# GDMCF/GDMCF

Measured on AMD Instinct MI355X. Metric: training users/sec, higher is better.
Workload: dtype f32; 1 GPU; yelp-shape synthetic rows, batch=400/GPU, dims=[1000], T=5, noise_scale=0.01, linear-var, mean_type=x0, reweight, AdamW lr=1e-5 (BASELINE configs[1]); n_items=34395, global_batch=400, parallelism=dp1, batch_rows=device CSR rows (CsrBatch)

## Files before the change

### gdmcf_amd/build.py

```python
import concurrent.futures
import hashlib
import os
import re
import subprocess
import sys

CSRC = os.path.join(os.path.dirname(os.path.abspath(__file__)), "csrc")
SOURCES = ["capi.hip", "dp_exchange.hip", "gemm_f32.hip", "gemm_bf16.hip", "gemm_split.hip", "gemm_small.hip", "gemm_dr.hip", "gemm_dr_tn.hip", "gemm_dr_fat.hip", "gemm_dr_kn.hip", "prep_input.hip", "noise.hip", "loss_tail.hip", "adamw.hip", "rows.hip", "reduce.hip", "linear.hip", "topk_spmm.hip", "spmm_bundle.hip", "score_topk.hip", "score_rank.hip", "bpr.hip", "cat.hip", "gather_fwd.hip", "ntxent.hip", "latent_step.hip", "cand_scores.hip", "rank.hip"]
HEADERS = ["common.h", "draws.h", "rank_order.h", "score_product.h", "gemm_dr.h", "gemm_epilogue.h", os.path.join("..", "..", "include", "gdmcf_hip.h")]
LIB = os.path.join(CSRC, "libgdmcf_hip.so")
ASM_LINT = ("gemm_dr_tn.hip", "gemm_split.hip")
STORE_LINT = ("gemm_f32.hip", "gemm_bf16.hip", "gemm_dr_fat.hip", "gemm_dr_kn.hip", "score_topk.hip", "score_rank.hip", "latent_step.hip")
NO_SPILL = ("gemm_f32.hip", "gemm_bf16.hip", "gemm_split.hip", "gemm_dr_tn.hip", "score_topk.hip", "score_rank.hip", "cat.hip", "gather_fwd.hip", "ntxent.hip", "latent_step.hip", "cand_scores.hip")
FLAGS = ["--offload-arch=gfx950", "-O3", "-std=c++17", "-fPIC", "-Wall", "-Wno-unused-function"]


def _hipcc():
    for c in (os.environ.get("HIPCC"), "/opt/rocm/bin/hipcc", "hipcc"):
        if c and (os.path.isabs(c) and os.path.exists(c) or not os.path.isabs(c)):
            return c
    raise RuntimeError("hipcc not found")


def _digest():
    h = hashlib.sha256()
    for f in SOURCES + HEADERS:
        with open(os.path.join(CSRC, f), "rb") as fh:
            h.update(fh.read())
    h.update(" ".join(FLAGS).encode())
    return h.hexdigest()


_REG = re.compile(r"\bv(\d+)\b|\bv\[(\d+):(\d+)\]")


def _regs(text):
    out = set()
    for m in _REG.finditer(text):
        if m.group(1) is not None:
            out.add(int(m.group(1)))
        else:
            out.update(range(int(m.group(2)), int(m.group(3)) + 1))
    return out


_SREG = re.compile(r"\bs(\d+)\b|\bs\[(\d+):(\d+)\]")


def _sregs(text):
    out = set()
    for m in _SREG.finditer(text):
        if m.group(1) is not None:
            out.add(int(m.group(1)))
        else:
            out.update(range(int(m.group(2)), int(m.group(3)) + 1))
    return out


def lint_ring_registers(asm_text, kernel_prefix="dr_tn_kernel"):
    bad, seen = [], 0
    for m in re.finditer(r"^(\S*%s\S*):[^\n]*\n(.*?)\n\s*s_endpgm" % kernel_prefix, asm_text, flags=re.S | re.M):
        name, body = m.group(1), m.group(2)
        seen += 1
        lines = [ln.split(";")[0].strip() for ln in body.splitlines()]
        lines = [ln for ln in lines if ln and not ln.endswith(":") and not ln.startswith(".")]
        ring = set()
        for ln in lines:
            if ln.startswith("buffer_load_dwordx4"):
                ring |= _regs(ln.split(",")[0])
        if not ring:
            bad.append(f"{name}: no asm ring loads found (lint out of date?)")
            continue
        first = next(i for i, ln in enumerate(lines) if ln.startswith("buffer_load_dwordx4"))
        drains = [i for i, ln in enumerate(lines) if ln.startswith("s_waitcnt") and "vmcnt(0)" in ln]
        last = drains[-1] if drains and drains[-1] > first else len(lines)
        for ln in lines[first:last]:
            mnem, _, ops = ln.partition(" ")
            parts = [o.strip() for o in ops.split(",")]
            if mnem.startswith("buffer_load_dwordx4"):
                if _regs(",".join(parts[1:])) & ring:
                    bad.append(f"{name}: ring register used as an address: {ln}")
            elif mnem.startswith("v_mfma"):
                if (_regs(parts[0]) | _regs(parts[3] if len(parts) > 3 else "")) & ring:
                    bad.append(f"{name}: MFMA accumulator inside the operand ring: {ln}")
            elif mnem.startswith(("v_mov", "v_pk_mov", "v_accvgpr", "scratch_", "v_swap")):
                if _regs(ops) & ring:
                    bad.append(f"{name}: copy or spill of a ring register: {ln}")
    if not seen:
        bad.append(f"no function named *{kernel_prefix}* in the assembly (lint out of date?)")
    return bad


_COPY = ("v_mov", "v_pk_mov", "v_accvgpr", "scratch_", "v_swap")
_VMEM = ("buffer_", "global_", "flat_", "scratch_")


def lint_vmcnt(asm_text, only=None):
    bad, nk = [], 0
    for m in re.finditer(r"^(_Z\S+):[^\n]*\n(.*?)\n\s*s_endpgm", asm_text, flags=re.S | re.M):
        name, body = m.group(1), m.group(2)
        if only and only not in name:
            continue
        ins, in_asm = [], False
        for ln in body.splitlines():
            t = ln.strip()
            if t.startswith(";;#ASMSTART"):
                in_asm = True
                continue
            if t.startswith(";;#ASMEND"):
                in_asm = False
                continue
            c = t.split(";")[0].strip()
            if not c or (c.startswith(".") and not c.endswith(":")):
                continue
            ins.append((c, in_asm))
        if not any(a and "load_dword" in c.split()[0] for c, a in ins):
            continue
        nk += 1
        leaders, labels = {0}, {}
        for k, (c, a) in enumerate(ins):
            if c.endswith(":"):
                labels[c[:-1]] = k
                leaders.add(k)
            elif c.startswith(("s_cbranch", "s_branch")):
                leaders.add(k + 1)
        starts = sorted(x for x in leaders if x < len(ins))
        blocks = [(st, starts[i + 1] if i + 1 < len(starts) else len(ins)) for i, st in enumerate(starts)]
        blk_of = {st: i for i, (st, en) in enumerate(blocks)}
        succ = []
        for bi, (st, en) in enumerate(blocks):
            mn, _, ops = ins[en - 1][0].partition(" ")
            nxt = []
            if mn.startswith(("s_cbranch", "s_branch")) and labels.get(ops.strip()) is not None:
                nxt.append(blk_of[labels[ops.strip()]])
            if not mn.startswith("s_branch") and bi + 1 < len(blocks):
                nxt.append(bi + 1)
            succ.append(nxt)
        found = {}

        def transfer(bi, st_in, report):
            st = dict(st_in)
            fresh = {}
            for k in range(*blocks[bi]):
                ln, a = ins[k]
                if ln.endswith(":"):
                    continue
                mnem, _, ops = ln.partition(" ")
                parts = [o.strip() for o in ops.split(",")]
                if a and mnem.startswith(_VMEM):
                    hot = _sregs(ops) & fresh.keys()
                    if hot and report:
                        found.setdefault(f"s{min(hot)} written by a VALU instruction < 5 wait states before this asm load reads it: {ln}", k)
                step = int(ops) + 1 if mnem == "s_nop" and ops.strip().isdigit() else 1
                fresh = {r: w - step for r, w in fresh.items() if w - step > 0}
                if mnem.startswith("v_") and parts and re.fullmatch(r"s\d+|s\[\d+:\d+\]", parts[0]):
                    for r in _sregs(parts[0]):
                        fresh[r] = 5
                if mnem == "s_waitcnt":
                    mm = re.search(r"vmcnt\((\d+)\)", ops)
                    if mm:
                        st = {r: rk for r, rk in st.items() if rk < int(mm.group(1))}
                    continue
                asm_load = a and "load_dword" in mnem
                touched = _regs(",".join(parts[1:]) if asm_load else ops) & st.keys()
                if touched and report:
                    what = "used as an address" if asm_load else ("copied / spilled" if mnem.startswith(_COPY) else "used")
                    found.setdefault(f"register v{min(touched)} {what} before a counted wait covers its load: {ln}", k)
                if mnem.startswith(_VMEM):
                    st = {r: min(rk + 1, 64) for r, rk in st.items()}
                    if asm_load:
                        for r in _regs(parts[0]):
                            st[r] = 0
            return st

        state = [None] * len(blocks)
        state[0] = {}
        work = [0]
        while work:
            bi = work.pop()
            out = transfer(bi, state[bi], False)
            for sj in succ[bi]:
                if state[sj] is None:
                    state[sj] = dict(out)
                    work.append(sj)
                else:
                    changed = False
                    for r, rk in out.items():
                        if state[sj].get(r, 65) > rk:
                            state[sj][r] = rk
                            changed = True
                    if changed:
                        work.append(sj)
        for bi in range(len(blocks)):
            if state[bi] is not None:
                transfer(bi, state[bi], True)
        bad += [f"{name}: {msg}" for msg, k in sorted(found.items(), key=lambda kv: kv[1])]
    if not nk:
        bad.append("no kernel with inline-asm loads in the assembly (lint out of date?)")
    return bad


def lint_store_data(asm_text):
    bad = []
    for m in re.finditer(r"^(_Z\S+):[^\n]*\n(.*?)\n\s*s_endpgm", asm_text, flags=re.S | re.M):
        name, body = m.group(1), m.group(2)
        lines = [ln.split(";")[0].strip() for ln in body.splitlines()]
        lines = [ln for ln in lines if ln and not ln.startswith(".") and not ln.endswith(":")]
        for k, ln in enumerate(lines):
            mnem, _, ops = ln.partition(" ")
            if not re.match(r"(buffer|global|flat|scratch)_store_dwordx[34]$", mnem):
                continue
            parts = [o.strip() for o in ops.split(",")]
            data = _regs(parts[1] if mnem.startswith(("global", "flat", "scratch")) else parts[0])
            left = 2
            for nxt in lines[k + 1:k + 8]:
                nm, _, nops = nxt.partition(" ")
                if nm == "s_nop":
                    left -= int(nops.strip() or 0) + 1
                else:
                    nparts = [o.strip() for o in nops.split(",")]
                    if nm.startswith("v_") and nparts and _regs(nparts[0]) & data and left > 0:
                        bad.append(f"{name}: data register of `{ln}` rewritten {2 - left} wait state(s) later by `{nxt}`")
                        break
                    left -= 1
                if left <= 0:
                    break
    return bad


def lint_fat_dma(asm_text, kernel="dr_fat_kernel"):
    bad, n_dma = [], 0
    for m in re.finditer(r"^(_Z\S*%s\S*):[^\n]*\n(.*?)\n\s*s_endpgm" % kernel, asm_text, flags=re.S | re.M):
        name, body = m.group(1), m.group(2)
        lines = [ln.split(";")[0].strip() for ln in body.splitlines()]
        lines = [ln for ln in lines if ln and (not ln.startswith(".") or ln.endswith(":"))]
        if not any(ln.startswith("buffer_load_dwordx4") and ln.endswith(" lds") for ln in lines):
            continue
        n_dma += 1
        pending = None
        for ln in lines:
            if ln.startswith("buffer_load_dwordx4") and ln.endswith(" lds"):
                pending = ln
            elif ln.startswith("s_waitcnt") and re.search(r"vmcnt\(0\)", ln):
                pending = None
            elif ln.startswith("ds_read_b128") and pending:
                bad.append(f"{name}: `{ln}` follows `{pending}` with no s_waitcnt vmcnt(0) in between")
                break
        loops, label, blk = 0, None, []
        for ln in lines + ["end:"]:
            if not ln.endswith(":"):
                blk.append(ln)
                continue
            if label and any(i.startswith("v_mfma") for i in blk) and any(
                    i.startswith(("s_cbranch", "s_branch")) and i.split()[-1] == label for i in blk):
                loops += 1
                moved = [i for i in blk if i.startswith(("scratch_", "v_accvgpr", "v_mov"))]
                if moved:
                    bad.append(f"{name}: {len(moved)} spill / move instruction(s) in the k loop, e.g. `{moved[0]}`")
            label, blk = ln[:-1], []
        if not loops:
            bad.append(f"{name}: no k loop found (lint out of date?)")
    if not n_dma:
        bad.append(f"no *{kernel}* with `buffer_load_dwordx4 ... lds` in the assembly (lint out of date?)")
    return bad


def build(force=False, verbose=True):
    stamp = os.path.join(CSRC, ".build_stamp")
    dig = _digest()
    if not force and os.path.exists(LIB) and os.path.exists(stamp) and open(stamp).read() == dig:
        return LIB
    hipcc = _hipcc()
    objs = []

    def compile_one(src):
        obj = os.path.join(CSRC, src.replace(".hip", ".o"))
        cmd = [hipcc] + FLAGS + ["-c", os.path.join(CSRC, src), "-o", obj]
        guarded = src in NO_SPILL
        if guarded:
            cmd.append("-Rpass-analysis=kernel-resource-usage")
        r = subprocess.run(cmd, capture_output=True, text=True)
        if r.returncode != 0:
            raise RuntimeError(f"hipcc failed for {src}:\n{r.stderr}")
        err = r.stderr
        if guarded:
            name, bad = None, []
            for line in err.splitlines():
                if "Function Name:" in line:
                    name = line.split("Function Name:")[1].split()[0]
                elif "VGPRs Spill:" in line and int(line.split("VGPRs Spill:")[1].split()[0]) > 0:
                    bad.append(name)
            if bad:
                raise RuntimeError(f"{src}: register spills in {len(bad)} kernel(s) with uncounted asm loads, e.g. {bad[0]}")
            err = err if ("warning:" in err or "error:" in err) else ""
        if verbose and err.strip():
            print(err, file=sys.stderr)
        if src in ASM_LINT or src in STORE_LINT:
            asm = os.path.join(CSRC, src.replace(".hip", ".lint.s"))
            r2 = subprocess.run([hipcc] + FLAGS + ["-S", "--cuda-device-only", os.path.join(CSRC, src), "-o", asm],
                                capture_output=True, text=True)
            if r2.returncode != 0:
                raise RuntimeError(f"hipcc -S failed for {src}:\n{r2.stderr}")
            text = open(asm).read()
            os.remove(asm)
            bad = lint_store_data(text)
            if src in ASM_LINT:
                bad += lint_vmcnt(text)
            if src == "gemm_dr_tn.hip":
                bad += lint_ring_registers(text)
            if src == "gemm_dr_fat.hip":
                bad += lint_fat_dma(text)
            if bad:
                raise RuntimeError(f"{src}: ISA lint failed (lint_store_data / lint_vmcnt / lint_ring_registers / lint_fat_dma):\n  " + "\n  ".join(bad[:12]))
        return obj

    with concurrent.futures.ThreadPoolExecutor(max_workers=min(8, len(SOURCES))) as ex:
        objs = list(ex.map(compile_one, SOURCES))
    cmd = [hipcc, "--offload-arch=gfx950", "-shared", "-fPIC", "-o", LIB] + objs
    r = subprocess.run(cmd, capture_output=True, text=True)
    if r.returncode != 0:
        raise RuntimeError(f"link failed:\n{r.stderr}")
    with open(stamp, "w") as fh:
        fh.write(dig)
    if verbose:
        print(f"built {LIB}")
    return LIB


if __name__ == "__main__":
    build(force="--force" in sys.argv)
```

### gdmcf_amd/csrc/gemm_dr.h

```cpp
#pragma once

#include "common.h"

namespace {
struct DrArgs {
    GdGemm g;
    int tiles_m, tiles_n, m_fastest;
    int ksp;
    int ctr;
    const GdAdamHyper* adam_dev;
    int stagger;
};
}

struct DrRoutes {
    bool dw;
    bool adamw;
    bool kn;
    bool fat;
    bool fat_slab;
};
DrRoutes& dr_routes();
int dr_cu_count();
int dr_stagger();

int gd_dr_tn_launch(GdGemm& g, hipStream_t s);
int gd_dr_kn_launch(GdGemm& g, hipStream_t s);
int gd_dr_fat_launch(int epi, GdGemm& g, hipStream_t s);
int gd_dr_fat_slab_launch(GdGemm& g, hipStream_t s);
```

### gdmcf_amd/csrc/gemm_dr.hip

```cpp
#include <stdlib.h>

#include "gemm_dr.h"

int dr_cu_count() {
    static int n_cu = 0;
    if (n_cu == 0) {
        int dev = 0;
        hipDeviceProp_t prop;
        n_cu = (hipGetDevice(&dev) == hipSuccess && hipGetDeviceProperties(&prop, dev) == hipSuccess) ? prop.multiProcessorCount : 256;
    }
    return n_cu;
}

#ifndef GD_FAT_SLAB_DEFAULT
#define GD_FAT_SLAB_DEFAULT 1
#endif

static bool dr_env_on(const char* name, bool dflt = true) {
    const char* v = getenv(name);
    return v == nullptr ? dflt : atoi(v) != 0;
}
DrRoutes& dr_routes() {
    static DrRoutes r = {dr_env_on("GDMCF_DR_DW"), dr_env_on("GDMCF_DR_ADAMW"), dr_env_on("GDMCF_DR_KN"), dr_env_on("GDMCF_DR_FAT"),
                         dr_env_on("GDMCF_DR_FAT_SLAB", GD_FAT_SLAB_DEFAULT != 0)};
    return r;
}

int dr_stagger() {
    static const int stagger = getenv("GDMCF_DR_STAGGER") ? atoi(getenv("GDMCF_DR_STAGGER")) : 3;
    return stagger;
}

int gd_gemm_dr_launch(int layA, int layB, int epi, GdGemm& g, hipStream_t s) {
    if (g.bf16) return GD_DR_NOT_TAKEN;
    if (g.accumulate || g.C16 || (g.splits > 1 && epi != GD_EPI_SLAB)) return GD_DR_NOT_TAKEN;
    if (layA == GD_LAY_MC && layB == GD_LAY_MC) {
        if (epi == GD_EPI_ADAMW) return gd_gemm_dr_adamw_multi(&g, 1, s);
        if (epi == GD_EPI_STORE) return gd_dr_tn_launch(g, s);
    } else if (layA == GD_LAY_KC && layB == GD_LAY_MC) {
        if (epi == GD_EPI_SLAB) return gd_dr_kn_launch(g, s);
    } else if (layA == GD_LAY_KC && layB == GD_LAY_KC) {
        if (epi == GD_EPI_LOSS || epi == GD_EPI_POST) return gd_dr_fat_launch(epi, g, s);
        if (epi == GD_EPI_SLAB) return gd_dr_fat_slab_launch(g, s);
    }
    return GD_DR_NOT_TAKEN;
}
```

### gdmcf_amd/csrc/gemm_dr_fat.hip

```cpp
#include <stdlib.h>

#include "gemm_dr.h"

#ifndef GD_FAT_DMA_DEFAULT
#define GD_FAT_DMA_DEFAULT 1
#endif

namespace {

template <int NB, int EPI, int DMA>
__global__ __launch_bounds__(256, 1) void dr_fat_kernel(const DrArgs d) {
    static_assert(EPI == GD_EPI_LOSS || EPI == GD_EPI_POST || EPI == GD_EPI_SLAB, "output layer with a fused epilogue, or split-K slabs");
    static_assert(NB >= 4 && NB <= 12, "5 x NB accumulator blocks must fit 256 registers");
    static_assert(DMA == 0 || DMA == 1, "B through staging registers, or straight into LDS");
    constexpr bool SLAB = EPI == GD_EPI_SLAB;
    typedef __attribute__((address_space(3))) void* lds_vp;
    constexpr int WAIT_VM0 = 0x0F70, WAIT_LGKM0 = 0xC07F;
    constexpr int TMB = 5;
    const GdGemm& g = d.g;
    const int lane = threadIdx.x & 63;
    const int wave = __builtin_amdgcn_readfirstlane(threadIdx.x >> 6);
    const int r = lane & 15, q = lane >> 4;
    extern __shared__ __attribute__((aligned(16))) float dr_lds[];
    float* const lds = dr_lds + wave * (2 * NB * 256);
    const int nblk = gridDim.x, per = nblk >> 3;
    const int wl = ((nblk & 7) == 0 ? ((int)(blockIdx.x & 7) * per + (int)(blockIdx.x >> 3)) : (int)blockIdx.x) * 4 + wave;
    const int n_waves = nblk * 4;
    const int ntiles = d.tiles_m * d.tiles_n;
    const __amdgpu_buffer_rsrc_t srdA = __builtin_amdgcn_make_buffer_rsrc(const_cast<float*>(g.A), 0, (int)(((int64_t)(g.M - 1) * g.lda + g.K) * 4), 0x00020000);
    const __amdgpu_buffer_rsrc_t srdB = __builtin_amdgcn_make_buffer_rsrc(const_cast<float*>(g.B), 0, (int)(((int64_t)(g.N - 1) * g.ldb + g.K) * 4), 0x00020000);
    const int NCH = d.ksp;
    const int c_mask = g.K >> 4;
    const int ntasks = SLAB ? ntiles * g.splits : ntiles;
    const int w_off = (lane >> 2) * 16 + (((lane & 3) ^ ((((lane >> 2) >> 2) & 1) << 1)) << 2);
    const int g_slot = DMA ? ((lane & 3) ^ ((((lane >> 2) >> 2) & 1) << 1)) : (lane & 3);
    const int r_off = r * 16 + ((q ^ (((r >> 2) & 1) << 1)) << 2);
    for (int task = wl; task < ntasks; task += n_waves) {
        const int split = SLAB ? task / ntiles : 0;
        const int tile = SLAB ? task - split * ntiles : task;
        const int c_lo = SLAB ? split * (g.kchunk >> 4) : 0;
        const int c_hi = SLAB ? min(c_lo + (g.kchunk >> 4), NCH) : NCH;
        const int c_in = SLAB ? min(c_hi, c_mask) : c_mask;
        const int tm = tile % d.tiles_m, tn = tile / d.tiles_m;
        const int m0 = tm * (16 * TMB), n0 = tn * (16 * NB);
        uint32_t offA[TMB], offB[NB];
#pragma unroll
        for (int i = 0; i < TMB; ++i) offA[i] = (uint32_t)((m0 + 16 * i + r) * g.lda + 4 * q) * 4u;
#pragma unroll
        for (int p = 0; p < NB; ++p) offB[p] = (uint32_t)(((int64_t)(n0 + 16 * p + (lane >> 2)) * g.ldb + 4 * g_slot) * 4);
        f32x4 acc[TMB][NB];
#pragma unroll
        for (int i = 0; i < TMB; ++i)
#pragma unroll
            for (int b = 0; b < NB; ++b) acc[i][b] = f32x4{0.f, 0.f, 0.f, 0.f};
        f32x4 xa[2][TMB], G[DMA ? 1 : NB], FB[NB];
        const int hp = DMA ? ((c_in - c_lo) & 1) : 0;
        const int k_lo = SLAB ? c_lo * 64 : 0;
        if (hp) {
#pragma unroll
            for (int i = 0; i < TMB; ++i) xa[1][i] = __builtin_bit_cast(f32x4, __builtin_amdgcn_raw_buffer_load_b128(srdA, offA[i], k_lo, 0));
        } else {
#pragma unroll
            for (int i = 0; i < TMB; ++i) xa[0][i] = __builtin_bit_cast(f32x4, __builtin_amdgcn_raw_buffer_load_b128(srdA, offA[i], k_lo, 0));
        }
        if constexpr (DMA) {
            __builtin_amdgcn_sched_barrier(0);
            __builtin_amdgcn_s_waitcnt(WAIT_LGKM0);
            __builtin_amdgcn_sched_barrier(0);
#pragma unroll
            for (int p = 0; p < NB; ++p) __builtin_amdgcn_raw_ptr_buffer_load_lds(srdB, (lds_vp)(lds + hp * (NB * 256) + p * 256), 16, (int)offB[p], k_lo, 0, 0);
        } else {
#pragma unroll
            for (int p = 0; p < NB; ++p) G[p] = __builtin_bit_cast(f32x4, __builtin_amdgcn_raw_buffer_load_b128(srdB, offB[p], k_lo, 0));
#pragma unroll
            for (int p = 0; p < NB; ++p) *reinterpret_cast<f32x4*>(lds + p * 256 + w_off) = G[p];
        }

#define GD_FAT_CHUNK(PAR, c, MSK)                                                                                         \
        {                                                                                                             \
             \
            const uint32_t kn = ((c) + 1 < c_hi) ? (uint32_t)((c) + 1) * 64u : 0x80000000u;                           \
            if constexpr (DMA) {                                                                                      \
                __builtin_amdgcn_sched_barrier(0);                                                                    \
                __builtin_amdgcn_s_waitcnt(WAIT_VM0);                                                                 \
                __builtin_amdgcn_sched_barrier(0);                                                                    \
            }                                                                                                         \
            _Pragma("unroll") for (int b = 0; b < NB; ++b)                                                            \
                FB[b] = *reinterpret_cast<const f32x4*>(lds + (PAR) * (NB * 256) + b * 256 + r_off);                  \
            if (MSK) {  \
                 \
                _Pragma("unroll") for (int e = 0; e < 4; ++e) {                                                       \
                    const bool keep = (c) * 16 + 4 * q + e < g.K;                                                     \
                    _Pragma("unroll") for (int i = 0; i < TMB; ++i) xa[PAR][i][e] = keep ? xa[PAR][i][e] : 0.f;       \
                    _Pragma("unroll") for (int b = 0; b < NB; ++b) FB[b][e] = keep ? FB[b][e] : 0.f;                  \
                }                                                                                                     \
            }                                                                                                         \
            __builtin_amdgcn_sched_barrier(0);                                                                        \
            _Pragma("unroll") for (int sx = 0; sx < 4; ++sx) {                                                        \
                _Pragma("unroll") for (int n = 0; n < TMB * NB; ++n) {                                                \
                    const int i = n / NB, b = n % NB;                                                                 \
                    if (sx == 0 && i == 0) asm volatile("" : "+v"(FB[b]));  \
                    if (sx == 0 && b == 0) asm volatile("" : "+v"(xa[PAR][i]));                                       \
                    acc[i][b] = __builtin_amdgcn_mfma_f32_16x16x4f32(xa[PAR][i][sx], FB[b][sx], acc[i][b], 0, 0, 0);  \
                     \
                    if (sx < 2 && n % 5 == 2) {      \
                        const int l = (sx == 0) ? n / 5 : NB + n / 5;                                                 \
                        if (l < TMB + NB) {                                                                           \
                            __builtin_amdgcn_sched_barrier(0);                                                        \
                            if (l < TMB)                                                                              \
                                xa[(PAR) ^ 1][l] = __builtin_bit_cast(f32x4, __builtin_amdgcn_raw_buffer_load_b128(   \
                                    srdA, offA[l], kn, 0));                                                           \
                            else if constexpr (DMA)                                                                   \
                                __builtin_amdgcn_raw_ptr_buffer_load_lds(                                             \
                                    srdB, (lds_vp)(lds + ((PAR) ^ 1) * (NB * 256) + (l - TMB) * 256), 16,             \
                                    (int)offB[l - TMB], (int)kn, 0, 0);                                               \
                            else                                                                                      \
                                G[l - TMB] = __builtin_bit_cast(f32x4, __builtin_amdgcn_raw_buffer_load_b128(         \
                                    srdB, offB[l - TMB], kn, 0));                                                     \
                            __builtin_amdgcn_sched_barrier(0);                                                        \
                        }                                                                                             \
                    }                                                                                                 \
                    if (!DMA && sx == 3 && n % 4 == 1 && n / 4 < NB) {  \
                        __builtin_amdgcn_sched_barrier(0);                                                            \
                        *reinterpret_cast<f32x4*>(lds + ((PAR) ^ 1) * (NB * 256) + (n / 4) * 256 + w_off) = G[n / 4]; \
                        __builtin_amdgcn_sched_barrier(0);                                                            \
                    }                                                                                                 \
                }                                                                                                     \
                __builtin_amdgcn_sched_barrier(0);                                                                    \
            }                                                                                                         \
        }
        const int c_pf = d.stagger > 0 ? ((NCH > d.stagger + 2 ? NCH - d.stagger : 0) & ~1) : -2;
        const int c_pairs = DMA ? c_in : c_hi;
        const int c_pfl = (DMA && c_pf >= 0) ? min(c_pf | hp, c_pairs - 2) : c_pf;
        int c = c_lo;
        if constexpr (DMA) {
            if (hp) {
                GD_FAT_CHUNK(1, c_lo, false);
                c = c_lo + 1;
            }
        }
        for (; c + 1 < c_pairs; c += 2) {
            if constexpr (EPI == GD_EPI_POST) {
                if (c == c_pfl) {
                    constexpr int NJL = (16 * NB * 4 + 127) / 128 + 1;
                    constexpr int NPI = (80 * NJL + 63) / 64;
                    float* const scratch = dr_lds + 4 * (2 * NB * 256) + wave * 64;
                    const __amdgpu_buffer_rsrc_t srdX = __builtin_amdgcn_make_buffer_rsrc(
                        const_cast<float*>(g.aux), 0, (int)(((int64_t)(g.M - 1) * g.ldaux + g.N) * 4), 0x00020000);
#pragma unroll
                    for (int pi = 0; pi < NPI; ++pi) {
                        const int t = min(pi * 64 + lane, 80 * NJL - 1);
                        const int row = min(m0 + t % 80, g.M - 1), j = t / 80;
                        const int col = min(j < NJL - 1 ? n0 + 32 * j : n0 + 16 * NB - 1, g.N - 1);
                        __builtin_amdgcn_raw_ptr_buffer_load_lds(srdX, (lds_vp)scratch, 4, (int)(((int64_t)row * g.ldaux + col) * 4), 0, 0, 0);
                    }
                }
            }
            if constexpr (DMA) {
                GD_FAT_CHUNK(0, c, false);
                GD_FAT_CHUNK(1, c + 1, false);
            } else {
                GD_FAT_CHUNK(0, c, c >= c_mask);
                GD_FAT_CHUNK(1, c + 1, c + 1 >= c_mask);
            }
        }
        if constexpr (DMA) {
            if (c < c_hi) GD_FAT_CHUNK(0, c, true);
        } else {
            if ((c_hi - c_lo) & 1) GD_FAT_CHUNK(0, c_hi - 1, c_hi - 1 >= c_mask);
        }
#undef GD_FAT_CHUNK
        if constexpr (DMA) {
            __builtin_amdgcn_sched_barrier(0);
            __builtin_amdgcn_s_waitcnt(WAIT_VM0);
            __builtin_amdgcn_sched_barrier(0);
        }

        if constexpr (SLAB) {
            constexpr int LDS_S = 16 * NB + 4, NJ_S = (4 * NB + 15) / 16;
            float* const slab = g.C + (int64_t)split * g.slab_stride;
#pragma unroll
            for (int i = 0; i < TMB; ++i) {
#pragma unroll
                for (int b = 0; b < NB; ++b)
#pragma unroll
                    for (int t = 0; t < 4; ++t) lds[(4 * q + t) * LDS_S + 16 * b + r] = acc[i][b][t];
                __builtin_amdgcn_sched_barrier(0);
#pragma unroll
                for (int p4 = 0; p4 < 4; ++p4) {
                    const int m = m0 + 16 * i + 4 * p4 + q;
#pragma unroll
                    for (int j = 0; j < NJ_S; ++j) {
                        const int c4 = r + 16 * j;
                        const int n = n0 + 4 * c4;
                        const f32x4 v = *reinterpret_cast<const f32x4*>(lds + (4 * p4 + q) * LDS_S + 4 * min(c4, 4 * NB - 1));
                        if (c4 < 4 * NB && m < g.M) {
                            if (n + 3 < g.N) {
                                *reinterpret_cast<f32x4*>(slab + (int64_t)m * g.ldc + n) = v;
                            } else {
                                for (int e = 0; e < 4 && n + e < g.N; ++e) slab[(int64_t)m * g.ldc + n + e] = v[e];
                            }
                        }
                    }
                }
                __builtin_amdgcn_sched_barrier(0);
            }
            continue;
        }

        constexpr int LDS_ = 16 * NB + 4;
        constexpr int NJ = (4 * NB + 15) / 16;
        typedef f32x4 f32x4_e __attribute__((aligned(4)));
        f32x4 bias4[NJ];
        int col4[NJ];
#pragma unroll
        for (int j = 0; j < NJ; ++j) {
            col4[j] = n0 + 4 * (r + 16 * j);
            bias4[j] = f32x4{0.f, 0.f, 0.f, 0.f};
            if (g.bias && r + 16 * j < 4 * NB) {
#pragma unroll
                for (int e = 0; e < 4; ++e) bias4[j][e] = g.bias[min(col4[j] + e, g.N - 1)];
            }
        }
        const bool has_z = (EPI == GD_EPI_POST) && (g.aux2 != nullptr);
        const bool has_r = (EPI == GD_EPI_POST) && (g.r2 != nullptr);
        struct Pre {
            f32x4 a[NJ], z[NJ];
            uint32_t w[NJ];
            float c1, c2, p1, p2, sg;
        } pre[2];
        auto fetch = [&](int i, int p4, Pre& P) {
            const int mc = min(m0 + 16 * i + 4 * p4 + q, g.M - 1);
            P.c1 = 1.f; P.c2 = 0.f; P.p1 = 0.f; P.p2 = 0.f; P.sg = 0.f;
            if (EPI == GD_EPI_LOSS) {
                if (g.r0) P.c1 = g.r0[mc];
            } else {
                P.c1 = g.r0[mc];
                P.c2 = g.r1[mc];
                if (has_r) { P.p1 = g.r2[mc]; P.p2 = g.r3[mc]; }
                if (has_z) P.sg = g.r4[mc];
            }
#pragma unroll
            for (int j = 0; j < NJ; ++j) {
                const int n = col4[j];
                const bool whole = (r + 16 * j < 4 * NB) && n + 3 < g.N;
                P.w[j] = 0u;
                P.a[j] = f32x4{0.f, 0.f, 0.f, 0.f};
                P.z[j] = f32x4{0.f, 0.f, 0.f, 0.f};
                if (EPI == GD_EPI_LOSS && g.aux_bits) {
                    P.w[j] = g.aux_bits[(int64_t)mc * g.ldbits + min((int64_t)(n >> 5), g.ldbits - 1)];
                } else if (whole) {
                    P.a[j] = *reinterpret_cast<const f32x4_e*>(g.aux + (int64_t)mc * g.ldaux + n);
                    if (has_z) P.z[j] = *reinterpret_cast<const f32x4_e*>(g.aux2 + (int64_t)mc * g.ldaux2 + n);
                }
            }
        };
        fetch(0, 0, pre[0]);
#pragma unroll
        for (int i = 0; i < TMB; ++i) {
#pragma unroll
            for (int b = 0; b < NB; ++b)
#pragma unroll
                for (int t = 0; t < 4; ++t) lds[(4 * q + t) * LDS_ + 16 * b + r] = acc[i][b][t];
            __builtin_amdgcn_sched_barrier(0);
#pragma unroll
            for (int p4 = 0; p4 < 4; ++p4) {
                const int step = 4 * i + p4;
                const Pre& P = pre[step & 1];
                if (step + 1 < 4 * TMB) fetch((step + 1) >> 2, (step + 1) & 3, pre[(step + 1) & 1]);
                const int m = m0 + 16 * i + 4 * p4 + q;
                const int mc = min(m, g.M - 1);
                const bool mok = m < g.M;
                float ss = 0.f;
                const float c1 = P.c1, c2 = P.c2, p1 = P.p1, p2 = P.p2, sg = P.sg;
#pragma unroll
                for (int j = 0; j < NJ; ++j) {
                    const int c4 = r + 16 * j;
                    const bool inb = c4 < 4 * NB;
                    const int n = col4[j];
                    const bool whole = inb && n + 3 < g.N;
                    const bool full = whole && mok;
                    const f32x4 v = *reinterpret_cast<const f32x4*>(lds + (4 * p4 + q) * LDS_ + 4 * min(c4, 4 * NB - 1));
                    f32x4 o, o2 = f32x4{0.f, 0.f, 0.f, 0.f};
                    if (EPI == GD_EPI_LOSS) {
                        f32x4 tg;
                        if (g.aux_bits) {
                            const uint32_t w = P.w[j] >> (n & 31);
#pragma unroll
                            for (int e = 0; e < 4; ++e) tg[e] = (float)((w >> e) & 1u);
                        } else if (whole) {
                            tg = P.a[j];
                        } else {
#pragma unroll
                            for (int e = 0; e < 4; ++e) tg[e] = g.aux[(int64_t)mc * g.ldaux + min(n + e, g.N - 1)];
                        }
#pragma unroll
                        for (int e = 0; e < 4; ++e) {
                            o2[e] = v[e] + bias4[j][e];
                            o[e] = c1 * o2[e] - tg[e];
                            if (inb && mok && n + e < g.N) ss += o[e] * o[e];
                        }
                    } else {
                        f32x4 xt = P.a[j], zz = P.z[j];
                        if (!whole) {
#pragma unroll
                            for (int e = 0; e < 4; ++e) {
                                xt[e] = g.aux[(int64_t)mc * g.ldaux + min(n + e, g.N - 1)];
                                if (has_z) zz[e] = g.aux2[(int64_t)mc * g.ldaux2 + min(n + e, g.N - 1)];
                            }
                        }
#pragma unroll
                        for (int e = 0; e < 4; ++e) {
                            const float vv = v[e] + bias4[j][e];
                            o2[e] = has_r ? (p1 * xt[e] - p2 * vv) : vv;
                            o[e] = c1 * o2[e] + c2 * xt[e];
                            if (has_z) o[e] += sg * zz[e];
                        }
                    }
                    if (full) {
                        *reinterpret_cast<f32x4_e*>(g.C + (int64_t)m * g.ldc + n) = o;
                        if (g.out2) *reinterpret_cast<f32x4_e*>(g.out2 + (int64_t)m * g.ldout2 + n) = o2;
                    } else if (inb && mok) {
                        for (int e = 0; e < 4 && n + e < g.N; ++e) {
                            g.C[(int64_t)m * g.ldc + n + e] = o[e];
                            if (g.out2) g.out2[(int64_t)m * g.ldout2 + n + e] = o2[e];
                        }
                    }
                }
                if (EPI == GD_EPI_LOSS) {
                    ss += __shfl_xor(ss, 1);
                    ss += __shfl_xor(ss, 2);
                    ss += __shfl_xor(ss, 4);
                    ss += __shfl_xor(ss, 8);
                    if (r == 0 && mok) g.rowpart[(int64_t)m * g.ld_rowpart + tn] = ss;
                }
                __builtin_amdgcn_sched_barrier(0);
            }
        }
    }
}

template <int NB>
int dr_fat_go(const DrArgs& d, int epi, int dma, int n_cu, hipStream_t s) {
    const size_t lds = (size_t)4 * 2 * NB * 256 * sizeof(float) + 4 * 64 * sizeof(float);
    void (*kern)(const DrArgs) =
        dma ? (epi == GD_EPI_SLAB ? dr_fat_kernel<NB, GD_EPI_SLAB, 1> : epi == GD_EPI_LOSS ? dr_fat_kernel<NB, GD_EPI_LOSS, 1> : dr_fat_kernel<NB, GD_EPI_POST, 1>)
            : (epi == GD_EPI_SLAB ? dr_fat_kernel<NB, GD_EPI_SLAB, 0> : epi == GD_EPI_LOSS ? dr_fat_kernel<NB, GD_EPI_LOSS, 0> : dr_fat_kernel<NB, GD_EPI_POST, 0>);
    static bool attr_set[6] = {false, false, false, false, false, false};
    const int ai = epi == GD_EPI_SLAB ? 4 + dma : 2 * dma + (epi == GD_EPI_LOSS);
    if (!attr_set[ai] && lds > 48 * 1024) {
        hipError_t e = hipFuncSetAttribute(reinterpret_cast<const void*>(kern), hipFuncAttributeMaxDynamicSharedMemorySize, (int)lds);
        if (e != hipSuccess) {
            gdmcf_set_error("hipFuncSetAttribute(dr_fat_kernel, LDS=%zu): %s", lds, hipGetErrorString(e));
            return GDMCF_E_HIP;
        }
        attr_set[ai] = true;
    }
    hipLaunchKernelGGL(kern, dim3(n_cu), dim3(256), lds, s, d);
    return GDMCF_OK;
}

int dr_fat_dma(const GdGemm& g) {
    static const int dma_env = getenv("GDMCF_FAT_DMA") ? atoi(getenv("GDMCF_FAT_DMA")) : GD_FAT_DMA_DEFAULT;
    return (dma_env > 0 && (reinterpret_cast<uintptr_t>(g.B) & 15) == 0 && (g.ldb & 3) == 0) ? 1 : 0;
}

}

int gd_dr_fat_launch(int epi, GdGemm& g, hipStream_t s) {
    if (!dr_routes().fat) return GD_DR_NOT_TAKEN;
    const int64_t lim = (int64_t)1 << 32;
    const int n_cu = dr_cu_count();
    const int tiles_m = gd_cdiv(g.M, 80);
    bool ok = (int64_t)g.M * g.lda * 4 < ((int64_t)1 << 31) && (int64_t)g.N * g.ldb * 4 < lim && g.lda >= g.K && g.ldb >= g.K &&
              g.K >= 256 && (long)tiles_m * 80 * 100 <= (long)g.M * 112 &&
              (n_cu & 7) == 0 && !(epi == GD_EPI_LOSS && g.rowpart == nullptr) &&
              !(epi == GD_EPI_LOSS && g.aux_bits && g.ldbits < (g.N + 31) / 32);
    int nb = 0;
    long best = 1L << 60;
    const long slots = 4L * n_cu;
    for (int c = 12; c >= 8 && ok; --c) {
        const long t = (long)tiles_m * gd_cdiv(g.N, 16 * c);
        const long cost = ((t + slots - 1) / slots) * c;
        if (t >= slots / 2 && cost < best) { best = cost; nb = c; }
    }
    if (ok && epi == GD_EPI_POST) {
        const long t128 = (long)gd_cdiv(g.M, 80) * gd_cdiv(g.N, 128);
        const long rounds = (t128 + 2 * n_cu - 1) / (2 * n_cu);
        if (t128 * 100 >= rounds * 2 * n_cu * 90) ok = false;
    }
    if (!ok || !nb || (epi == GD_EPI_LOSS && g.ld_rowpart < gd_cdiv(g.N, 16 * nb))) return GD_DR_NOT_TAKEN;
    DrArgs d = {};
    d.tiles_m = tiles_m;
    d.tiles_n = gd_cdiv(g.N, 16 * nb);
    d.m_fastest = 1;
    d.ksp = gd_cdiv(g.K, 16);
    {
        static const int pf = getenv("GDMCF_FAT_PF") ? atoi(getenv("GDMCF_FAT_PF")) : 10;
        d.stagger = pf;
    }
    const int dma = dr_fat_dma(g);
    g.tiles_m = d.tiles_m;
    g.tiles_n = d.tiles_n;
    d.g = g;
    d.ctr = 0;
    int rc = GDMCF_OK;
    {
        GdProfScope prof(g.prof_tag, 2.0 * g.M * g.N * g.K, s);
        switch (nb) {
            case 8: rc = dr_fat_go<8>(d, epi, dma, n_cu, s); break;
            case 9: rc = dr_fat_go<9>(d, epi, dma, n_cu, s); break;
            case 10: rc = dr_fat_go<10>(d, epi, dma, n_cu, s); break;
            case 11: rc = dr_fat_go<11>(d, epi, dma, n_cu, s); break;
            default: rc = dr_fat_go<12>(d, epi, dma, n_cu, s); break;
        }
    }
    if (rc != GDMCF_OK) return rc;
    t_gd_last_gemm = 4;
    return gd_launch_status("gemm_dr");
}

int gd_dr_fat_slab_plan(int M, int N, int K, int* nb_out, int* cps_out) {
    if (!dr_routes().fat_slab || M <= 0 || N < 128 || K < 4096) return 0;
    const int n_cu = dr_cu_count();
    const int tiles_m = gd_cdiv(M, 80);
    if ((n_cu & 7) != 0 || (long)tiles_m * 80 * 100 > (long)M * 112) return 0;
    const long slots = 4L * n_cu;
    const int chunks = gd_cdiv(K, 16);
    int nb = 0, cps = 0;
    long best = 1L << 60;
    for (int c = 8; c <= 12; ++c) {
        const long tiles = (long)tiles_m * gd_cdiv(N, 16 * c);
        if (tiles > slots) continue;
        long sp = slots / tiles;
        if (sp > chunks / 8) sp = chunks / 8;
        if (sp > 64) sp = 64;
        if (sp < 2) continue;
        const int per = gd_cdiv(chunks, (int)sp);
        if ((long)c * per < best) { best = (long)c * per; nb = c; cps = per; }
    }
    if (!nb) return 0;
    if (nb_out) *nb_out = nb;
    if (cps_out) *cps_out = cps;
    return gd_cdiv(chunks, cps);
}

int gd_dr_fat_slab_launch(GdGemm& g, hipStream_t s) {
    int nb = 0, cps = 0;
    const int splits = gd_dr_fat_slab_plan(g.M, g.N, g.K, &nb, &cps);
    if (!splits) return GD_DR_NOT_TAKEN;
    const size_t need = (size_t)splits * g.M * g.ldc * sizeof(float);
    const bool ok = gd_aligned16(g.C) && (g.ldc & 3) == 0 && g.ldc >= g.N &&
                    g.ws_cap >= need && g.slab_stride >= (int64_t)g.M * g.ldc && (g.slab_stride & 3) == 0 &&
                    (int64_t)g.M * g.lda * 4 < ((int64_t)1 << 31) && (int64_t)g.N * g.ldb * 4 < ((int64_t)1 << 32) && g.lda >= g.K && g.ldb >= g.K;
    if (!ok) return GD_DR_NOT_TAKEN;
    const int n_cu = dr_cu_count();
    DrArgs d = {};
    d.tiles_m = gd_cdiv(g.M, 80);
    d.tiles_n = gd_cdiv(g.N, 16 * nb);
    d.m_fastest = 1;
    d.ksp = gd_cdiv(g.K, 16);
    g.splits = splits;
    g.kchunk = cps * 16;
    g.tiles_m = d.tiles_m;
    g.tiles_n = d.tiles_n;
    d.g = g;
    d.ctr = 0;
    const int dma = dr_fat_dma(g);
    int rc = GDMCF_OK;
    {
        GdProfScope prof(g.prof_tag, 2.0 * g.M * g.N * g.K, s);
        switch (nb) {
            case 8: rc = dr_fat_go<8>(d, GD_EPI_SLAB, dma, n_cu, s); break;
            case 9: rc = dr_fat_go<9>(d, GD_EPI_SLAB, dma, n_cu, s); break;
            case 10: rc = dr_fat_go<10>(d, GD_EPI_SLAB, dma, n_cu, s); break;
            case 11: rc = dr_fat_go<11>(d, GD_EPI_SLAB, dma, n_cu, s); break;
            default: rc = dr_fat_go<12>(d, GD_EPI_SLAB, dma, n_cu, s); break;
        }
    }
    if (rc != GDMCF_OK) return rc;
    t_gd_last_gemm = 6;
    return gd_launch_status("gemm_dr_fat_slab");
}
```

Before: 321,100 users/s.

## Specialize fat GEMM epilogues by feature flags and split into separate compilation units

Moves the fat output-layer GEMM kernel into a shared header and adds a template flag parameter that selects specialized LOSS/POST epilogue variants, including an interior-tile fast path and software-prefetched per-row epilogue operands. The instantiations are split across new source files so they compile in parallel. The aim is to cut branching and the exposed latency of global loads in the fused epilogue for the output layer. In exchange it brings more template instantiations, longer build times and a larger code size, and the epilogue logic is duplicated across variants.

```diff
diff --git a/gdmcf_amd/build.py b/gdmcf_amd/build.py
--- a/gdmcf_amd/build.py
+++ b/gdmcf_amd/build.py
@@ -6,11 +6,11 @@
 import sys
 
 CSRC = os.path.join(os.path.dirname(os.path.abspath(__file__)), "csrc")
-SOURCES = ["capi.hip", "dp_exchange.hip", "gemm_f32.hip", "gemm_bf16.hip", "gemm_split.hip", "gemm_small.hip", "gemm_dr.hip", "gemm_dr_tn.hip", "gemm_dr_fat.hip", "gemm_dr_kn.hip", "prep_input.hip", "noise.hip", "loss_tail.hip", "adamw.hip", "rows.hip", "reduce.hip", "linear.hip", "topk_spmm.hip", "spmm_bundle.hip", "score_topk.hip", "score_rank.hip", "bpr.hip", "cat.hip", "gather_fwd.hip", "ntxent.hip", "latent_step.hip", "cand_scores.hip", "rank.hip"]
-HEADERS = ["common.h", "draws.h", "rank_order.h", "score_product.h", "gemm_dr.h", "gemm_epilogue.h", os.path.join("..", "..", "include", "gdmcf_hip.h")]
+SOURCES = ["capi.hip", "dp_exchange.hip", "gemm_f32.hip", "gemm_bf16.hip", "gemm_split.hip", "gemm_small.hip", "gemm_dr.hip", "gemm_dr_tn.hip", "gemm_dr_fat.hip", "gemm_dr_fat_loss.hip", "gemm_dr_fat_post.hip", "gemm_dr_fat_post2.hip", "gemm_dr_kn.hip", "prep_input.hip", "noise.hip", "loss_tail.hip", "adamw.hip", "rows.hip", "reduce.hip", "linear.hip", "topk_spmm.hip", "spmm_bundle.hip", "score_topk.hip", "score_rank.hip", "bpr.hip", "cat.hip", "gather_fwd.hip", "ntxent.hip", "latent_step.hip", "cand_scores.hip", "rank.hip"]
+HEADERS = ["common.h", "draws.h", "rank_order.h", "score_product.h", "gemm_dr.h", "gemm_dr_fat_kernel.h", "gemm_epilogue.h", os.path.join("..", "..", "include", "gdmcf_hip.h")]
 LIB = os.path.join(CSRC, "libgdmcf_hip.so")
 ASM_LINT = ("gemm_dr_tn.hip", "gemm_split.hip")
-STORE_LINT = ("gemm_f32.hip", "gemm_bf16.hip", "gemm_dr_fat.hip", "gemm_dr_kn.hip", "score_topk.hip", "score_rank.hip", "latent_step.hip")
+STORE_LINT = ("gemm_f32.hip", "gemm_bf16.hip", "gemm_dr_fat.hip", "gemm_dr_fat_loss.hip", "gemm_dr_fat_post.hip", "gemm_dr_fat_post2.hip", "gemm_dr_kn.hip", "score_topk.hip", "score_rank.hip", "latent_step.hip")
 NO_SPILL = ("gemm_f32.hip", "gemm_bf16.hip", "gemm_split.hip", "gemm_dr_tn.hip", "score_topk.hip", "score_rank.hip", "cat.hip", "gather_fwd.hip", "ntxent.hip", "latent_step.hip", "cand_scores.hip")
 FLAGS = ["--offload-arch=gfx950", "-O3", "-std=c++17", "-fPIC", "-Wall", "-Wno-unused-function"]
 
@@ -308,7 +308,7 @@
                 bad += lint_vmcnt(text)
             if src == "gemm_dr_tn.hip":
                 bad += lint_ring_registers(text)
-            if src == "gemm_dr_fat.hip":
+            if src.startswith("gemm_dr_fat"):
                 bad += lint_fat_dma(text)
             if bad:
                 raise RuntimeError(f"{src}: ISA lint failed (lint_store_data / lint_vmcnt / lint_ring_registers / lint_fat_dma):\n  " + "\n  ".join(bad[:12]))
diff --git a/gdmcf_amd/csrc/gemm_dr.h b/gdmcf_amd/csrc/gemm_dr.h
--- a/gdmcf_amd/csrc/gemm_dr.h
+++ b/gdmcf_amd/csrc/gemm_dr.h
@@ -10,6 +10,7 @@
     int ctr;
     const GdAdamHyper* adam_dev;
     int stagger;
+    int interior;
 };
 }
 
@@ -19,6 +20,7 @@
     bool kn;
     bool fat;
     bool fat_slab;
+    bool fat_epi;
 };
 DrRoutes& dr_routes();
 int dr_cu_count();
diff --git a/gdmcf_amd/csrc/gemm_dr.hip b/gdmcf_amd/csrc/gemm_dr.hip
--- a/gdmcf_amd/csrc/gemm_dr.hip
+++ b/gdmcf_amd/csrc/gemm_dr.hip
@@ -16,13 +16,17 @@
 #define GD_FAT_SLAB_DEFAULT 1
 #endif
 
+#ifndef GD_FAT_EPI_DEFAULT
+#define GD_FAT_EPI_DEFAULT 1
+#endif
+
 static bool dr_env_on(const char* name, bool dflt = true) {
     const char* v = getenv(name);
     return v == nullptr ? dflt : atoi(v) != 0;
 }
 DrRoutes& dr_routes() {
     static DrRoutes r = {dr_env_on("GDMCF_DR_DW"), dr_env_on("GDMCF_DR_ADAMW"), dr_env_on("GDMCF_DR_KN"), dr_env_on("GDMCF_DR_FAT"),
-                         dr_env_on("GDMCF_DR_FAT_SLAB", GD_FAT_SLAB_DEFAULT != 0)};
+                         dr_env_on("GDMCF_DR_FAT_SLAB", GD_FAT_SLAB_DEFAULT != 0), dr_env_on("GDMCF_FAT_EPI", GD_FAT_EPI_DEFAULT != 0)};
     return r;
 }
 
diff --git a/gdmcf_amd/csrc/gemm_dr_fat.hip b/gdmcf_amd/csrc/gemm_dr_fat.hip
--- a/gdmcf_amd/csrc/gemm_dr_fat.hip
+++ b/gdmcf_amd/csrc/gemm_dr_fat.hip
@@ -1,6 +1,6 @@
 #include <stdlib.h>
 
-#include "gemm_dr.h"
+#include "gemm_dr_fat_kernel.h"
 
 #ifndef GD_FAT_DMA_DEFAULT
 #define GD_FAT_DMA_DEFAULT 1
@@ -8,356 +8,11 @@
 
 namespace {
 
-template <int NB, int EPI, int DMA>
-__global__ __launch_bounds__(256, 1) void dr_fat_kernel(const DrArgs d) {
-    static_assert(EPI == GD_EPI_LOSS || EPI == GD_EPI_POST || EPI == GD_EPI_SLAB, "output layer with a fused epilogue, or split-K slabs");
-    static_assert(NB >= 4 && NB <= 12, "5 x NB accumulator blocks must fit 256 registers");
-    static_assert(DMA == 0 || DMA == 1, "B through staging registers, or straight into LDS");
-    constexpr bool SLAB = EPI == GD_EPI_SLAB;
-    typedef __attribute__((address_space(3))) void* lds_vp;
-    constexpr int WAIT_VM0 = 0x0F70, WAIT_LGKM0 = 0xC07F;
-    constexpr int TMB = 5;
-    const GdGemm& g = d.g;
-    const int lane = threadIdx.x & 63;
-    const int wave = __builtin_amdgcn_readfirstlane(threadIdx.x >> 6);
-    const int r = lane & 15, q = lane >> 4;
-    extern __shared__ __attribute__((aligned(16))) float dr_lds[];
-    float* const lds = dr_lds + wave * (2 * NB * 256);
-    const int nblk = gridDim.x, per = nblk >> 3;
-    const int wl = ((nblk & 7) == 0 ? ((int)(blockIdx.x & 7) * per + (int)(blockIdx.x >> 3)) : (int)blockIdx.x) * 4 + wave;
-    const int n_waves = nblk * 4;
-    const int ntiles = d.tiles_m * d.tiles_n;
-    const __amdgpu_buffer_rsrc_t srdA = __builtin_amdgcn_make_buffer_rsrc(const_cast<float*>(g.A), 0, (int)(((int64_t)(g.M - 1) * g.lda + g.K) * 4), 0x00020000);
-    const __amdgpu_buffer_rsrc_t srdB = __builtin_amdgcn_make_buffer_rsrc(const_cast<float*>(g.B), 0, (int)(((int64_t)(g.N - 1) * g.ldb + g.K) * 4), 0x00020000);
-    const int NCH = d.ksp;
-    const int c_mask = g.K >> 4;
-    const int ntasks = SLAB ? ntiles * g.splits : ntiles;
-    const int w_off = (lane >> 2) * 16 + (((lane & 3) ^ ((((lane >> 2) >> 2) & 1) << 1)) << 2);
-    const int g_slot = DMA ? ((lane & 3) ^ ((((lane >> 2) >> 2) & 1) << 1)) : (lane & 3);
-    const int r_off = r * 16 + ((q ^ (((r >> 2) & 1) << 1)) << 2);
-    for (int task = wl; task < ntasks; task += n_waves) {
-        const int split = SLAB ? task / ntiles : 0;
-        const int tile = SLAB ? task - split * ntiles : task;
-        const int c_lo = SLAB ? split * (g.kchunk >> 4) : 0;
-        const int c_hi = SLAB ? min(c_lo + (g.kchunk >> 4), NCH) : NCH;
-        const int c_in = SLAB ? min(c_hi, c_mask) : c_mask;
-        const int tm = tile % d.tiles_m, tn = tile / d.tiles_m;
-        const int m0 = tm * (16 * TMB), n0 = tn * (16 * NB);
-        uint32_t offA[TMB], offB[NB];
-#pragma unroll
-        for (int i = 0; i < TMB; ++i) offA[i] = (uint32_t)((m0 + 16 * i + r) * g.lda + 4 * q) * 4u;
-#pragma unroll
-        for (int p = 0; p < NB; ++p) offB[p] = (uint32_t)(((int64_t)(n0 + 16 * p + (lane >> 2)) * g.ldb + 4 * g_slot) * 4);
-        f32x4 acc[TMB][NB];
-#pragma unroll
-        for (int i = 0; i < TMB; ++i)
-#pragma unroll
-            for (int b = 0; b < NB; ++b) acc[i][b] = f32x4{0.f, 0.f, 0.f, 0.f};
-        f32x4 xa[2][TMB], G[DMA ? 1 : NB], FB[NB];
-        const int hp = DMA ? ((c_in - c_lo) & 1) : 0;
-        const int k_lo = SLAB ? c_lo * 64 : 0;
-        if (hp) {
-#pragma unroll
-            for (int i = 0; i < TMB; ++i) xa[1][i] = __builtin_bit_cast(f32x4, __builtin_amdgcn_raw_buffer_load_b128(srdA, offA[i], k_lo, 0));
-        } else {
-#pragma unroll
-            for (int i = 0; i < TMB; ++i) xa[0][i] = __builtin_bit_cast(f32x4, __builtin_amdgcn_raw_buffer_load_b128(srdA, offA[i], k_lo, 0));
-        }
-        if constexpr (DMA) {
-            __builtin_amdgcn_sched_barrier(0);
-            __builtin_amdgcn_s_waitcnt(WAIT_LGKM0);
-            __builtin_amdgcn_sched_barrier(0);
-#pragma unroll
-            for (int p = 0; p < NB; ++p) __builtin_amdgcn_raw_ptr_buffer_load_lds(srdB, (lds_vp)(lds + hp * (NB * 256) + p * 256), 16, (int)offB[p], k_lo, 0, 0);
-        } else {
-#pragma unroll
-            for (int p = 0; p < NB; ++p) G[p] = __builtin_bit_cast(f32x4, __builtin_amdgcn_raw_buffer_load_b128(srdB, offB[p], k_lo, 0));
-#pragma unroll
-            for (int p = 0; p < NB; ++p) *reinterpret_cast<f32x4*>(lds + p * 256 + w_off) = G[p];
-        }
-
-#define GD_FAT_CHUNK(PAR, c, MSK)                                                                                         \
-        {                                                                                                             \
-             \
-            const uint32_t kn = ((c) + 1 < c_hi) ? (uint32_t)((c) + 1) * 64u : 0x80000000u;                           \
-            if constexpr (DMA) {                                                                                      \
-                __builtin_amdgcn_sched_barrier(0);                                                                    \
-                __builtin_amdgcn_s_waitcnt(WAIT_VM0);                                                                 \
-                __builtin_amdgcn_sched_barrier(0);                                                                    \
-            }                                                                                                         \
-            _Pragma("unroll") for (int b = 0; b < NB; ++b)                                                            \
-                FB[b] = *reinterpret_cast<const f32x4*>(lds + (PAR) * (NB * 256) + b * 256 + r_off);                  \
-            if (MSK) {  \
-                 \
-                _Pragma("unroll") for (int e = 0; e < 4; ++e) {                                                       \
-                    const bool keep = (c) * 16 + 4 * q + e < g.K;                                                     \
-                    _Pragma("unroll") for (int i = 0; i < TMB; ++i) xa[PAR][i][e] = keep ? xa[PAR][i][e] : 0.f;       \
-                    _Pragma("unroll") for (int b = 0; b < NB; ++b) FB[b][e] = keep ? FB[b][e] : 0.f;                  \
-                }                                                                                                     \
-            }                                                                                                         \
-            __builtin_amdgcn_sched_barrier(0);                                                                        \
-            _Pragma("unroll") for (int sx = 0; sx < 4; ++sx) {                                                        \
-                _Pragma("unroll") for (int n = 0; n < TMB * NB; ++n) {                                                \
-                    const int i = n / NB, b = n % NB;                                                                 \
-                    if (sx == 0 && i == 0) asm volatile("" : "+v"(FB[b]));  \
-                    if (sx == 0 && b == 0) asm volatile("" : "+v"(xa[PAR][i]));                                       \
-                    acc[i][b] = __builtin_amdgcn_mfma_f32_16x16x4f32(xa[PAR][i][sx], FB[b][sx], acc[i][b], 0, 0, 0);  \
-                     \
-                    if (sx < 2 && n % 5 == 2) {      \
-                        const int l = (sx == 0) ? n / 5 : NB + n / 5;                                                 \
-                        if (l < TMB + NB) {                                                                           \
-                            __builtin_amdgcn_sched_barrier(0);                                                        \
-                            if (l < TMB)                                                                              \
-                                xa[(PAR) ^ 1][l] = __builtin_bit_cast(f32x4, __builtin_amdgcn_raw_buffer_load_b128(   \
-                                    srdA, offA[l], kn, 0));                                                           \
-                            else if constexpr (DMA)                                                                   \
-                                __builtin_amdgcn_raw_ptr_buffer_load_lds(                                             \
-                                    srdB, (lds_vp)(lds + ((PAR) ^ 1) * (NB * 256) + (l - TMB) * 256), 16,             \
-                                    (int)offB[l - TMB], (int)kn, 0, 0);                                               \
-                            else                                                                                      \
-                                G[l - TMB] = __builtin_bit_cast(f32x4, __builtin_amdgcn_raw_buffer_load_b128(         \
-                                    srdB, offB[l - TMB], kn, 0));                                                     \
-                            __builtin_amdgcn_sched_barrier(0);                                                        \
-                        }                                                                                             \
-                    }                                                                                                 \
-                    if (!DMA && sx == 3 && n % 4 == 1 && n / 4 < NB) {  \
-                        __builtin_amdgcn_sched_barrier(0);                                                            \
-                        *reinterpret_cast<f32x4*>(lds + ((PAR) ^ 1) * (NB * 256) + (n / 4) * 256 + w_off) = G[n / 4]; \
-                        __builtin_amdgcn_sched_barrier(0);                                                            \
-                    }                                                                                                 \
-                }                                                                                                     \
-                __builtin_amdgcn_sched_barrier(0);                                                                    \
-            }                                                                                                         \
-        }
-        const int c_pf = d.stagger > 0 ? ((NCH > d.stagger + 2 ? NCH - d.stagger : 0) & ~1) : -2;
-        const int c_pairs = DMA ? c_in : c_hi;
-        const int c_pfl = (DMA && c_pf >= 0) ? min(c_pf | hp, c_pairs - 2) : c_pf;
-        int c = c_lo;
-        if constexpr (DMA) {
-            if (hp) {
-                GD_FAT_CHUNK(1, c_lo, false);
-                c = c_lo + 1;
-            }
-        }
-        for (; c + 1 < c_pairs; c += 2) {
-            if constexpr (EPI == GD_EPI_POST) {
-                if (c == c_pfl) {
-                    constexpr int NJL = (16 * NB * 4 + 127) / 128 + 1;
-                    constexpr int NPI = (80 * NJL + 63) / 64;
-                    float* const scratch = dr_lds + 4 * (2 * NB * 256) + wave * 64;
-                    const __amdgpu_buffer_rsrc_t srdX = __builtin_amdgcn_make_buffer_rsrc(
-                        const_cast<float*>(g.aux), 0, (int)(((int64_t)(g.M - 1) * g.ldaux + g.N) * 4), 0x00020000);
-#pragma unroll
-                    for (int pi = 0; pi < NPI; ++pi) {
-                        const int t = min(pi * 64 + lane, 80 * NJL - 1);
-                        const int row = min(m0 + t % 80, g.M - 1), j = t / 80;
-                        const int col = min(j < NJL - 1 ? n0 + 32 * j : n0 + 16 * NB - 1, g.N - 1);
-                        __builtin_amdgcn_raw_ptr_buffer_load_lds(srdX, (lds_vp)scratch, 4, (int)(((int64_t)row * g.ldaux + col) * 4), 0, 0, 0);
-                    }
-                }
-            }
-            if constexpr (DMA) {
-                GD_FAT_CHUNK(0, c, false);
-                GD_FAT_CHUNK(1, c + 1, false);
-            } else {
-                GD_FAT_CHUNK(0, c, c >= c_mask);
-                GD_FAT_CHUNK(1, c + 1, c + 1 >= c_mask);
-            }
-        }
-        if constexpr (DMA) {
-            if (c < c_hi) GD_FAT_CHUNK(0, c, true);
-        } else {
-            if ((c_hi - c_lo) & 1) GD_FAT_CHUNK(0, c_hi - 1, c_hi - 1 >= c_mask);
-        }
-#undef GD_FAT_CHUNK
-        if constexpr (DMA) {
-            __builtin_amdgcn_sched_barrier(0);
-            __builtin_amdgcn_s_waitcnt(WAIT_VM0);
-            __builtin_amdgcn_sched_barrier(0);
-        }
-
-        if constexpr (SLAB) {
-            constexpr int LDS_S = 16 * NB + 4, NJ_S = (4 * NB + 15) / 16;
-            float* const slab = g.C + (int64_t)split * g.slab_stride;
-#pragma unroll
-            for (int i = 0; i < TMB; ++i) {
-#pragma unroll
-                for (int b = 0; b < NB; ++b)
-#pragma unroll
-                    for (int t = 0; t < 4; ++t) lds[(4 * q + t) * LDS_S + 16 * b + r] = acc[i][b][t];
-                __builtin_amdgcn_sched_barrier(0);
-#pragma unroll
-                for (int p4 = 0; p4 < 4; ++p4) {
-                    const int m = m0 + 16 * i + 4 * p4 + q;
-#pragma unroll
-                    for (int j = 0; j < NJ_S; ++j) {
-                        const int c4 = r + 16 * j;
-                        const int n = n0 + 4 * c4;
-                        const f32x4 v = *reinterpret_cast<const f32x4*>(lds + (4 * p4 + q) * LDS_S + 4 * min(c4, 4 * NB - 1));
-                        if (c4 < 4 * NB && m < g.M) {
-                            if (n + 3 < g.N) {
-                                *reinterpret_cast<f32x4*>(slab + (int64_t)m * g.ldc + n) = v;
-                            } else {
-                                for (int e = 0; e < 4 && n + e < g.N; ++e) slab[(int64_t)m * g.ldc + n + e] = v[e];
-                            }
-                        }
-                    }
-                }
-                __builtin_amdgcn_sched_barrier(0);
-            }
-            continue;
-        }
-
-        constexpr int LDS_ = 16 * NB + 4;
-        constexpr int NJ = (4 * NB + 15) / 16;
-        typedef f32x4 f32x4_e __attribute__((aligned(4)));
-        f32x4 bias4[NJ];
-        int col4[NJ];
-#pragma unroll
-        for (int j = 0; j < NJ; ++j) {
-            col4[j] = n0 + 4 * (r + 16 * j);
-            bias4[j] = f32x4{0.f, 0.f, 0.f, 0.f};
-            if (g.bias && r + 16 * j < 4 * NB) {
-#pragma unroll
-                for (int e = 0; e < 4; ++e) bias4[j][e] = g.bias[min(col4[j] + e, g.N - 1)];
-            }
-        }
-        const bool has_z = (EPI == GD_EPI_POST) && (g.aux2 != nullptr);
-        const bool has_r = (EPI == GD_EPI_POST) && (g.r2 != nullptr);
-        struct Pre {
-            f32x4 a[NJ], z[NJ];
-            uint32_t w[NJ];
-            float c1, c2, p1, p2, sg;
-        } pre[2];
-        auto fetch = [&](int i, int p4, Pre& P) {
-            const int mc = min(m0 + 16 * i + 4 * p4 + q, g.M - 1);
-            P.c1 = 1.f; P.c2 = 0.f; P.p1 = 0.f; P.p2 = 0.f; P.sg = 0.f;
-            if (EPI == GD_EPI_LOSS) {
-                if (g.r0) P.c1 = g.r0[mc];
-            } else {
-                P.c1 = g.r0[mc];
-                P.c2 = g.r1[mc];
-                if (has_r) { P.p1 = g.r2[mc]; P.p2 = g.r3[mc]; }
-                if (has_z) P.sg = g.r4[mc];
-            }
-#pragma unroll
-            for (int j = 0; j < NJ; ++j) {
-                const int n = col4[j];
-                const bool whole = (r + 16 * j < 4 * NB) && n + 3 < g.N;
-                P.w[j] = 0u;
-                P.a[j] = f32x4{0.f, 0.f, 0.f, 0.f};
-                P.z[j] = f32x4{0.f, 0.f, 0.f, 0.f};
-                if (EPI == GD_EPI_LOSS && g.aux_bits) {
-                    P.w[j] = g.aux_bits[(int64_t)mc * g.ldbits + min((int64_t)(n >> 5), g.ldbits - 1)];
-                } else if (whole) {
-                    P.a[j] = *reinterpret_cast<const f32x4_e*>(g.aux + (int64_t)mc * g.ldaux + n);
-                    if (has_z) P.z[j] = *reinterpret_cast<const f32x4_e*>(g.aux2 + (int64_t)mc * g.ldaux2 + n);
-                }
-            }
-        };
-        fetch(0, 0, pre[0]);
-#pragma unroll
-        for (int i = 0; i < TMB; ++i) {
-#pragma unroll
-            for (int b = 0; b < NB; ++b)
-#pragma unroll
-                for (int t = 0; t < 4; ++t) lds[(4 * q + t) * LDS_ + 16 * b + r] = acc[i][b][t];
-            __builtin_amdgcn_sched_barrier(0);
-#pragma unroll
-            for (int p4 = 0; p4 < 4; ++p4) {
-                const int step = 4 * i + p4;
-                const Pre& P = pre[step & 1];
-                if (step + 1 < 4 * TMB) fetch((step + 1) >> 2, (step + 1) & 3, pre[(step + 1) & 1]);
-                const int m = m0 + 16 * i + 4 * p4 + q;
-                const int mc = min(m, g.M - 1);
-                const bool mok = m < g.M;
-                float ss = 0.f;
-                const float c1 = P.c1, c2 = P.c2, p1 = P.p1, p2 = P.p2, sg = P.sg;
-#pragma unroll
-                for (int j = 0; j < NJ; ++j) {
-                    const int c4 = r + 16 * j;
-                    const bool inb = c4 < 4 * NB;
-                    const int n = col4[j];
-                    const bool whole = inb && n + 3 < g.N;
-                    const bool full = whole && mok;
-                    const f32x4 v = *reinterpret_cast<const f32x4*>(lds + (4 * p4 + q) * LDS_ + 4 * min(c4, 4 * NB - 1));
-                    f32x4 o, o2 = f32x4{0.f, 0.f, 0.f, 0.f};
-                    if (EPI == GD_EPI_LOSS) {
-                        f32x4 tg;
-                        if (g.aux_bits) {
-                            const uint32_t w = P.w[j] >> (n & 31);
-#pragma unroll
-                            for (int e = 0; e < 4; ++e) tg[e] = (float)((w >> e) & 1u);
-                        } else if (whole) {
-                            tg = P.a[j];
-                        } else {
-#pragma unroll
-                            for (int e = 0; e < 4; ++e) tg[e] = g.aux[(int64_t)mc * g.ldaux + min(n + e, g.N - 1)];
-                        }
-#pragma unroll
-                        for (int e = 0; e < 4; ++e) {
-                            o2[e] = v[e] + bias4[j][e];
-                            o[e] = c1 * o2[e] - tg[e];
-                            if (inb && mok && n + e < g.N) ss += o[e] * o[e];
-                        }
-                    } else {
-                        f32x4 xt = P.a[j], zz = P.z[j];
-                        if (!whole) {
-#pragma unroll
-                            for (int e = 0; e < 4; ++e) {
-                                xt[e] = g.aux[(int64_t)mc * g.ldaux + min(n + e, g.N - 1)];
-                                if (has_z) zz[e] = g.aux2[(int64_t)mc * g.ldaux2 + min(n + e, g.N - 1)];
-                            }
-                        }
-#pragma unroll
-                        for (int e = 0; e < 4; ++e) {
-                            const float vv = v[e] + bias4[j][e];
-                            o2[e] = has_r ? (p1 * xt[e] - p2 * vv) : vv;
-                            o[e] = c1 * o2[e] + c2 * xt[e];
-                            if (has_z) o[e] += sg * zz[e];
-                        }
-                    }
-                    if (full) {
-                        *reinterpret_cast<f32x4_e*>(g.C + (int64_t)m * g.ldc + n) = o;
-                        if (g.out2) *reinterpret_cast<f32x4_e*>(g.out2 + (int64_t)m * g.ldout2 + n) = o2;
-                    } else if (inb && mok) {
-                        for (int e = 0; e < 4 && n + e < g.N; ++e) {
-                            g.C[(int64_t)m * g.ldc + n + e] = o[e];
-                            if (g.out2) g.out2[(int64_t)m * g.ldout2 + n + e] = o2[e];
-                        }
-                    }
-                }
-                if (EPI == GD_EPI_LOSS) {
-                    ss += __shfl_xor(ss, 1);
-                    ss += __shfl_xor(ss, 2);
-                    ss += __shfl_xor(ss, 4);
-                    ss += __shfl_xor(ss, 8);
-                    if (r == 0 && mok) g.rowpart[(int64_t)m * g.ld_rowpart + tn] = ss;
-                }
-                __builtin_amdgcn_sched_barrier(0);
-            }
-        }
-    }
-}
-
-template <int NB>
-int dr_fat_go(const DrArgs& d, int epi, int dma, int n_cu, hipStream_t s) {
-    const size_t lds = (size_t)4 * 2 * NB * 256 * sizeof(float) + 4 * 64 * sizeof(float);
-    void (*kern)(const DrArgs) =
-        dma ? (epi == GD_EPI_SLAB ? dr_fat_kernel<NB, GD_EPI_SLAB, 1> : epi == GD_EPI_LOSS ? dr_fat_kernel<NB, GD_EPI_LOSS, 1> : dr_fat_kernel<NB, GD_EPI_POST, 1>)
-            : (epi == GD_EPI_SLAB ? dr_fat_kernel<NB, GD_EPI_SLAB, 0> : epi == GD_EPI_LOSS ? dr_fat_kernel<NB, GD_EPI_LOSS, 0> : dr_fat_kernel<NB, GD_EPI_POST, 0>);
-    static bool attr_set[6] = {false, false, false, false, false, false};
-    const int ai = epi == GD_EPI_SLAB ? 4 + dma : 2 * dma + (epi == GD_EPI_LOSS);
-    if (!attr_set[ai] && lds > 48 * 1024) {
-        hipError_t e = hipFuncSetAttribute(reinterpret_cast<const void*>(kern), hipFuncAttributeMaxDynamicSharedMemorySize, (int)lds);
-        if (e != hipSuccess) {
-            gdmcf_set_error("hipFuncSetAttribute(dr_fat_kernel, LDS=%zu): %s", lds, hipGetErrorString(e));
-            return GDMCF_E_HIP;
-        }
-        attr_set[ai] = true;
-    }
-    hipLaunchKernelGGL(kern, dim3(n_cu), dim3(256), lds, s, d);
-    return GDMCF_OK;
+int dr_fat_go(int nb, const DrArgs& d, int epi, int dma, int n_cu, hipStream_t s) {
+    if (epi == GD_EPI_SLAB) return dma ? dr_fat_start_nb<GD_EPI_SLAB, 1, 0>(nb, d, n_cu, s) : dr_fat_start_nb<GD_EPI_SLAB, 0, 0>(nb, d, n_cu, s);
+    if (epi == GD_EPI_LOSS)
+        return dma ? dr_fat_start_nb<GD_EPI_LOSS, 1, GD_FAT_GENERIC>(nb, d, n_cu, s) : dr_fat_start_nb<GD_EPI_LOSS, 0, GD_FAT_GENERIC>(nb, d, n_cu, s);
+    return dr_fat_start_nb<GD_EPI_POST, 0, GD_FAT_GENERIC>(nb, d, n_cu, s);
 }
 
 int dr_fat_dma(const GdGemm& g) {
@@ -407,12 +62,14 @@
     int rc = GDMCF_OK;
     {
         GdProfScope prof(g.prof_tag, 2.0 * g.M * g.N * g.K, s);
-        switch (nb) {
-            case 8: rc = dr_fat_go<8>(d, epi, dma, n_cu, s); break;
-            case 9: rc = dr_fat_go<9>(d, epi, dma, n_cu, s); break;
-            case 10: rc = dr_fat_go<10>(d, epi, dma, n_cu, s); break;
-            case 11: rc = dr_fat_go<11>(d, epi, dma, n_cu, s); break;
-            default: rc = dr_fat_go<12>(d, epi, dma, n_cu, s); break;
+        d.interior = dr_routes().fat_epi ? 1 : 0;
+        if (dma && epi == GD_EPI_LOSS && g.out2 == nullptr) {
+            rc = gd_dr_fat_loss_start(nb, g.aux_bits ? 1 : 0, &d, n_cu, s);
+        } else if (dma && epi == GD_EPI_POST) {
+            const int fl = (g.r2 ? 1 : 0) | (g.aux2 ? 2 : 0) | (g.out2 ? 4 : 0);
+            rc = fl < 4 ? gd_dr_fat_post_start(nb, fl, &d, n_cu, s) : gd_dr_fat_post2_start(nb, fl, &d, n_cu, s);
+        } else {
+            rc = dr_fat_go(nb, d, epi, dma, n_cu, s);
         }
     }
     if (rc != GDMCF_OK) return rc;
@@ -470,13 +127,7 @@
     int rc = GDMCF_OK;
     {
         GdProfScope prof(g.prof_tag, 2.0 * g.M * g.N * g.K, s);
-        switch (nb) {
-            case 8: rc = dr_fat_go<8>(d, GD_EPI_SLAB, dma, n_cu, s); break;
-            case 9: rc = dr_fat_go<9>(d, GD_EPI_SLAB, dma, n_cu, s); break;
-            case 10: rc = dr_fat_go<10>(d, GD_EPI_SLAB, dma, n_cu, s); break;
-            case 11: rc = dr_fat_go<11>(d, GD_EPI_SLAB, dma, n_cu, s); break;
-            default: rc = dr_fat_go<12>(d, GD_EPI_SLAB, dma, n_cu, s); break;
-        }
+        rc = dr_fat_go(nb, d, GD_EPI_SLAB, dma, n_cu, s);
     }
     if (rc != GDMCF_OK) return rc;
     t_gd_last_gemm = 6;
diff --git a/gdmcf_amd/csrc/gemm_dr_fat_kernel.h b/gdmcf_amd/csrc/gemm_dr_fat_kernel.h
--- /dev/null
+++ b/gdmcf_amd/csrc/gemm_dr_fat_kernel.h
@@ -0,0 +1,529 @@
+#pragma once
+
+#include "gemm_dr.h"
+
+#ifndef GD_FAT_EPI_PROBE
+#define GD_FAT_EPI_PROBE 5
+#endif
+
+namespace {
+
+constexpr int GD_FAT_GENERIC = -1;
+
+template <int SH>
+__device__ __forceinline__ float fat_row_shl(float x) {
+    return __builtin_bit_cast(float, __builtin_amdgcn_update_dpp(0, __builtin_bit_cast(int, x), 0x100 + SH, 0xF, 0xF, true));
+}
+
+__device__ __forceinline__ float fat_sq_add(float ss, float o) {
+#pragma clang fp contract(off)
+    return ss + o * o;
+}
+
+__device__ __forceinline__ float fat_post_elem(float vv, float xt, float zz, float c1, float c2, float p1, float p2, float sg, bool has_r,
+                                               bool has_z, float& o2) {
+#pragma clang fp contract(off)
+    o2 = has_r ? (p1 * xt - p2 * vv) : vv;
+    float o = __builtin_fmaf(c2, xt, c1 * o2);
+    if (has_z) o = __builtin_fmaf(sg, zz, o);
+    return o;
+}
+
+template <int NB, int EPI, int DMA, int FL>
+__global__ __launch_bounds__(256, 1) void dr_fat_kernel(const DrArgs d) {
+    static_assert(EPI == GD_EPI_LOSS || EPI == GD_EPI_POST || EPI == GD_EPI_SLAB, "output layer with a fused epilogue, or split-K slabs");
+    static_assert(NB >= 4 && NB <= 12, "5 x NB accumulator blocks must fit 256 registers");
+    static_assert(DMA == 0 || DMA == 1, "B through staging registers, or straight into LDS");
+    static_assert(FL >= GD_FAT_GENERIC && FL < (EPI == GD_EPI_POST ? 8 : EPI == GD_EPI_LOSS ? 2 : 1), "epilogue flavour");
+    constexpr bool SLAB = EPI == GD_EPI_SLAB;
+    constexpr bool GEN = FL == GD_FAT_GENERIC;
+    typedef __attribute__((address_space(3))) void* lds_vp;
+    constexpr int WAIT_VM0 = 0x0F70, WAIT_LGKM0 = 0xC07F;
+    constexpr int TMB = 5;
+    const GdGemm& g = d.g;
+    const int lane = threadIdx.x & 63;
+    const int wave = __builtin_amdgcn_readfirstlane(threadIdx.x >> 6);
+    const int r = lane & 15, q = lane >> 4;
+    extern __shared__ __attribute__((aligned(16))) float dr_lds[];
+    float* const lds = dr_lds + wave * (2 * NB * 256);
+    const int nblk = gridDim.x, per = nblk >> 3;
+    const int wl = ((nblk & 7) == 0 ? ((int)(blockIdx.x & 7) * per + (int)(blockIdx.x >> 3)) : (int)blockIdx.x) * 4 + wave;
+    const int n_waves = nblk * 4;
+    const int ntiles = d.tiles_m * d.tiles_n;
+    const __amdgpu_buffer_rsrc_t srdA = __builtin_amdgcn_make_buffer_rsrc(const_cast<float*>(g.A), 0, (int)(((int64_t)(g.M - 1) * g.lda + g.K) * 4), 0x00020000);
+    const __amdgpu_buffer_rsrc_t srdB = __builtin_amdgcn_make_buffer_rsrc(const_cast<float*>(g.B), 0, (int)(((int64_t)(g.N - 1) * g.ldb + g.K) * 4), 0x00020000);
+    const int NCH = d.ksp;
+    const int c_mask = g.K >> 4;
+    const int ntasks = SLAB ? ntiles * g.splits : ntiles;
+    const int w_off = (lane >> 2) * 16 + (((lane & 3) ^ ((((lane >> 2) >> 2) & 1) << 1)) << 2);
+    const int g_slot = DMA ? ((lane & 3) ^ ((((lane >> 2) >> 2) & 1) << 1)) : (lane & 3);
+    const int r_off = r * 16 + ((q ^ (((r >> 2) & 1) << 1)) << 2);
+    for (int task = wl; task < ntasks; task += n_waves) {
+        const int split = SLAB ? task / ntiles : 0;
+        const int tile = SLAB ? task - split * ntiles : task;
+        const int c_lo = SLAB ? split * (g.kchunk >> 4) : 0;
+        const int c_hi = SLAB ? min(c_lo + (g.kchunk >> 4), NCH) : NCH;
+        const int c_in = SLAB ? min(c_hi, c_mask) : c_mask;
+        const int tm = tile % d.tiles_m, tn = tile / d.tiles_m;
+        const int m0 = tm * (16 * TMB), n0 = tn * (16 * NB);
+        uint32_t offA[TMB], offB[NB];
+#pragma unroll
+        for (int i = 0; i < TMB; ++i) offA[i] = (uint32_t)((m0 + 16 * i + r) * g.lda + 4 * q) * 4u;
+#pragma unroll
+        for (int p = 0; p < NB; ++p) offB[p] = (uint32_t)(((int64_t)(n0 + 16 * p + (lane >> 2)) * g.ldb + 4 * g_slot) * 4);
+        f32x4 acc[TMB][NB];
+#pragma unroll
+        for (int i = 0; i < TMB; ++i)
+#pragma unroll
+            for (int b = 0; b < NB; ++b) acc[i][b] = f32x4{0.f, 0.f, 0.f, 0.f};
+        f32x4 xa[2][TMB], G[DMA ? 1 : NB], FB[NB];
+        const int hp = DMA ? ((c_in - c_lo) & 1) : 0;
+        const int k_lo = SLAB ? c_lo * 64 : 0;
+        if (hp) {
+#pragma unroll
+            for (int i = 0; i < TMB; ++i) xa[1][i] = __builtin_bit_cast(f32x4, __builtin_amdgcn_raw_buffer_load_b128(srdA, offA[i], k_lo, 0));
+        } else {
+#pragma unroll
+            for (int i = 0; i < TMB; ++i) xa[0][i] = __builtin_bit_cast(f32x4, __builtin_amdgcn_raw_buffer_load_b128(srdA, offA[i], k_lo, 0));
+        }
+        if constexpr (DMA) {
+            __builtin_amdgcn_sched_barrier(0);
+            __builtin_amdgcn_s_waitcnt(WAIT_LGKM0);
+            __builtin_amdgcn_sched_barrier(0);
+#pragma unroll
+            for (int p = 0; p < NB; ++p) __builtin_amdgcn_raw_ptr_buffer_load_lds(srdB, (lds_vp)(lds + hp * (NB * 256) + p * 256), 16, (int)offB[p], k_lo, 0, 0);
+        } else {
+#pragma unroll
+            for (int p = 0; p < NB; ++p) G[p] = __builtin_bit_cast(f32x4, __builtin_amdgcn_raw_buffer_load_b128(srdB, offB[p], k_lo, 0));
+#pragma unroll
+            for (int p = 0; p < NB; ++p) *reinterpret_cast<f32x4*>(lds + p * 256 + w_off) = G[p];
+        }
+
+#define GD_FAT_CHUNK(PAR, c, MSK)                                                                                         \
+        {                                                                                                             \
+             \
+            const uint32_t kn = ((c) + 1 < c_hi) ? (uint32_t)((c) + 1) * 64u : 0x80000000u;                           \
+            if constexpr (DMA) {                                                                                      \
+                __builtin_amdgcn_sched_barrier(0);                                                                    \
+                __builtin_amdgcn_s_waitcnt(WAIT_VM0);                                                                 \
+                __builtin_amdgcn_sched_barrier(0);                                                                    \
+            }                                                                                                         \
+            _Pragma("unroll") for (int b = 0; b < NB; ++b)                                                            \
+                FB[b] = *reinterpret_cast<const f32x4*>(lds + (PAR) * (NB * 256) + b * 256 + r_off);                  \
+            if (MSK) {  \
+                 \
+                _Pragma("unroll") for (int e = 0; e < 4; ++e) {                                                       \
+                    const bool keep = (c) * 16 + 4 * q + e < g.K;                                                     \
+                    _Pragma("unroll") for (int i = 0; i < TMB; ++i) xa[PAR][i][e] = keep ? xa[PAR][i][e] : 0.f;       \
+                    _Pragma("unroll") for (int b = 0; b < NB; ++b) FB[b][e] = keep ? FB[b][e] : 0.f;                  \
+                }                                                                                                     \
+            }                                                                                                         \
+            __builtin_amdgcn_sched_barrier(0);                                                                        \
+            _Pragma("unroll") for (int sx = 0; sx < 4; ++sx) {                                                        \
+                _Pragma("unroll") for (int n = 0; n < TMB * NB; ++n) {                                                \
+                    const int i = n / NB, b = n % NB;                                                                 \
+                    if (sx == 0 && i == 0) asm volatile("" : "+v"(FB[b]));  \
+                    if (sx == 0 && b == 0) asm volatile("" : "+v"(xa[PAR][i]));                                       \
+                    acc[i][b] = __builtin_amdgcn_mfma_f32_16x16x4f32(xa[PAR][i][sx], FB[b][sx], acc[i][b], 0, 0, 0);  \
+                     \
+                    if (sx < 2 && n % 5 == 2) {      \
+                        const int l = (sx == 0) ? n / 5 : NB + n / 5;                                                 \
+                        if (l < TMB + NB) {                                                                           \
+                            __builtin_amdgcn_sched_barrier(0);                                                        \
+                            if (l < TMB)                                                                              \
+                                xa[(PAR) ^ 1][l] = __builtin_bit_cast(f32x4, __builtin_amdgcn_raw_buffer_load_b128(   \
+                                    srdA, offA[l], kn, 0));                                                           \
+                            else if constexpr (DMA)                                                                   \
+                                __builtin_amdgcn_raw_ptr_buffer_load_lds(                                             \
+                                    srdB, (lds_vp)(lds + ((PAR) ^ 1) * (NB * 256) + (l - TMB) * 256), 16,             \
+                                    (int)offB[l - TMB], (int)kn, 0, 0);                                               \
+                            else                                                                                      \
+                                G[l - TMB] = __builtin_bit_cast(f32x4, __builtin_amdgcn_raw_buffer_load_b128(         \
+                                    srdB, offB[l - TMB], kn, 0));                                                     \
+                            __builtin_amdgcn_sched_barrier(0);                                                        \
+                        }                                                                                             \
+                    }                                                                                                 \
+                    if (!DMA && sx == 3 && n % 4 == 1 && n / 4 < NB) {  \
+                        __builtin_amdgcn_sched_barrier(0);                                                            \
+                        *reinterpret_cast<f32x4*>(lds + ((PAR) ^ 1) * (NB * 256) + (n / 4) * 256 + w_off) = G[n / 4]; \
+                        __builtin_amdgcn_sched_barrier(0);                                                            \
+                    }                                                                                                 \
+                }                                                                                                     \
+                __builtin_amdgcn_sched_barrier(0);                                                                    \
+            }                                                                                                         \
+        }
+        const int c_pf = d.stagger > 0 ? ((NCH > d.stagger + 2 ? NCH - d.stagger : 0) & ~1) : -2;
+        const int c_pairs = DMA ? c_in : c_hi;
+        const int c_pfl = (DMA && c_pf >= 0) ? min(c_pf | hp, c_pairs - 2) : c_pf;
+        int c = c_lo;
+        if constexpr (DMA) {
+            if (hp) {
+                GD_FAT_CHUNK(1, c_lo, false);
+                c = c_lo + 1;
+            }
+        }
+        for (; c + 1 < c_pairs; c += 2) {
+            if constexpr (EPI == GD_EPI_POST) {
+                if (c == c_pfl) {
+                    constexpr int NJL = (16 * NB * 4 + 127) / 128 + 1;
+                    constexpr int NPI = (80 * NJL + 63) / 64;
+                    float* const scratch = dr_lds + 4 * (2 * NB * 256) + wave * 64;
+                    const __amdgpu_buffer_rsrc_t srdX = __builtin_amdgcn_make_buffer_rsrc(
+                        const_cast<float*>(g.aux), 0, (int)(((int64_t)(g.M - 1) * g.ldaux + g.N) * 4), 0x00020000);
+#pragma unroll
+                    for (int pi = 0; pi < NPI; ++pi) {
+                        const int t = min(pi * 64 + lane, 80 * NJL - 1);
+                        const int row = min(m0 + t % 80, g.M - 1), j = t / 80;
+                        const int col = min(j < NJL - 1 ? n0 + 32 * j : n0 + 16 * NB - 1, g.N - 1);
+                        __builtin_amdgcn_raw_ptr_buffer_load_lds(srdX, (lds_vp)scratch, 4, (int)(((int64_t)row * g.ldaux + col) * 4), 0, 0, 0);
+                    }
+                }
+            }
+            if constexpr (DMA) {
+                GD_FAT_CHUNK(0, c, false);
+                GD_FAT_CHUNK(1, c + 1, false);
+            } else {
+                GD_FAT_CHUNK(0, c, c >= c_mask);
+                GD_FAT_CHUNK(1, c + 1, c + 1 >= c_mask);
+            }
+        }
+        if constexpr (DMA) {
+            if (c < c_hi) GD_FAT_CHUNK(0, c, true);
+        } else {
+            if ((c_hi - c_lo) & 1) GD_FAT_CHUNK(0, c_hi - 1, c_hi - 1 >= c_mask);
+        }
+#undef GD_FAT_CHUNK
+        if constexpr (DMA) {
+            __builtin_amdgcn_sched_barrier(0);
+            __builtin_amdgcn_s_waitcnt(WAIT_VM0);
+            __builtin_amdgcn_sched_barrier(0);
+        }
+
+        if constexpr (SLAB) {
+            constexpr int LDS_S = 16 * NB + 4, NJ_S = (4 * NB + 15) / 16;
+            float* const slab = g.C + (int64_t)split * g.slab_stride;
+#pragma unroll
+            for (int i = 0; i < TMB; ++i) {
+#pragma unroll
+                for (int b = 0; b < NB; ++b)
+#pragma unroll
+                    for (int t = 0; t < 4; ++t) lds[(4 * q + t) * LDS_S + 16 * b + r] = acc[i][b][t];
+                __builtin_amdgcn_sched_barrier(0);
+#pragma unroll
+                for (int p4 = 0; p4 < 4; ++p4) {
+                    const int m = m0 + 16 * i + 4 * p4 + q;
+#pragma unroll
+                    for (int j = 0; j < NJ_S; ++j) {
+                        const int c4 = r + 16 * j;
+                        const int n = n0 + 4 * c4;
+                        const f32x4 v = *reinterpret_cast<const f32x4*>(lds + (4 * p4 + q) * LDS_S + 4 * min(c4, 4 * NB - 1));
+                        if (c4 < 4 * NB && m < g.M) {
+                            if (n + 3 < g.N) {
+                                *reinterpret_cast<f32x4*>(slab + (int64_t)m * g.ldc + n) = v;
+                            } else {
+                                for (int e = 0; e < 4 && n + e < g.N; ++e) slab[(int64_t)m * g.ldc + n + e] = v[e];
+                            }
+                        }
+                    }
+                }
+                __builtin_amdgcn_sched_barrier(0);
+            }
+            continue;
+        }
+
+        constexpr int LDS_ = 16 * NB + 4;
+        constexpr int NJ = (4 * NB + 15) / 16;
+        typedef f32x4 f32x4_e __attribute__((aligned(4)));
+        f32x4 bias4[NJ];
+        int col4[NJ];
+#pragma unroll
+        for (int j = 0; j < NJ; ++j) {
+            col4[j] = n0 + 4 * (r + 16 * j);
+            bias4[j] = f32x4{0.f, 0.f, 0.f, 0.f};
+            if (g.bias && r + 16 * j < 4 * NB) {
+#pragma unroll
+                for (int e = 0; e < 4; ++e) bias4[j][e] = g.bias[min(col4[j] + e, g.N - 1)];
+            }
+        }
+        const bool has_z = (EPI == GD_EPI_POST) && (GEN ? g.aux2 != nullptr : (FL & 2) != 0);
+        const bool has_r = (EPI == GD_EPI_POST) && (GEN ? g.r2 != nullptr : (FL & 1) != 0);
+        const bool bits = (EPI == GD_EPI_LOSS) && (GEN ? g.aux_bits != nullptr : (FL & 1) != 0);
+        const bool out2 = GEN ? g.out2 != nullptr : ((EPI == GD_EPI_POST) && (FL & 4) != 0);
+
+        if constexpr (!GEN) {
+            if (d.interior && m0 + 16 * TMB <= g.M && n0 + 16 * NB <= g.N) {
+                constexpr bool LOSS = EPI == GD_EPI_LOSS;
+                constexpr bool F_BITS = LOSS && (FL & 1), F_R = !LOSS && (FL & 1), F_Z = !LOSS && (FL & 2), F_O2 = !LOSS && (FL & 4);
+                constexpr int PRB = GD_FAT_EPI_PROBE;
+                struct PreI {
+                    f32x4 a[NJ], z[NJ];
+                    uint32_t w[NJ];
+                    float c1, c2, p1, p2, sg;
+                } pin[2];
+                auto own = [&](int j) { return 16 * (j + 1) <= 4 * NB || r + 16 * j < 4 * NB; };
+                auto fetch_in = [&](int step, PreI& P) {
+                    const int64_t m = m0 + 4 * step + q;
+                    if constexpr (LOSS) {
+                        P.c1 = 1.f;
+                        if (g.r0) P.c1 = g.r0[m];
+                    } else {
+                        P.c1 = g.r0[m];
+                        P.c2 = g.r1[m];
+                        if constexpr (F_R) { P.p1 = g.r2[m]; P.p2 = g.r3[m]; }
+                        if constexpr (F_Z) P.sg = g.r4[m];
+                    }
+#pragma unroll
+                    for (int j = 0; j < NJ; ++j) {
+                        if (!own(j)) continue;
+                        const int n = col4[j];
+                        if constexpr (F_BITS) {
+                            P.w[j] = g.aux_bits[m * g.ldbits + (n >> 5)];
+                        } else {
+                            P.a[j] = *reinterpret_cast<const f32x4_e*>(g.aux + m * g.ldaux + n);
+                            if constexpr (F_Z) P.z[j] = *reinterpret_cast<const f32x4_e*>(g.aux2 + m * g.ldaux2 + n);
+                        }
+                    }
+                };
+                if constexpr (PRB == 1) {
+#pragma unroll
+                    for (int i = 0; i < TMB; ++i)
+#pragma unroll
+                        for (int b = 0; b < NB; ++b) asm volatile("" ::"v"(acc[i][b]));
+                    continue;
+                }
+                if constexpr (PRB >= 3) fetch_in(0, pin[0]);
+#pragma unroll
+                for (int i = 0; i < TMB; ++i) {
+#pragma unroll
+                    for (int b = 0; b < NB; ++b)
+#pragma unroll
+                        for (int t = 0; t < 4; ++t) lds[(4 * q + t) * LDS_ + 16 * b + r] = acc[i][b][t];
+                    __builtin_amdgcn_sched_barrier(0);
+                    float ss[4] = {0.f, 0.f, 0.f, 0.f};
+#pragma unroll
+                    for (int p4 = 0; p4 < 4; ++p4) {
+                        const int step = 4 * i + p4;
+                        const PreI& P = pin[step & 1];
+                        if (PRB >= 3 && step + 1 < 4 * TMB) fetch_in(step + 1, pin[(step + 1) & 1]);
+                        const int64_t m = m0 + 4 * step + q;
+#pragma unroll
+                        for (int j = 0; j < NJ; ++j) {
+                            if (!own(j)) continue;
+                            const int n = col4[j];
+                            const f32x4 v = *reinterpret_cast<const f32x4*>(lds + (4 * p4 + q) * LDS_ + 4 * (r + 16 * j));
+                            f32x4 o, o2;
+                            if constexpr (PRB < 4) {
+                                o = v;
+                                o2 = v;
+                                if constexpr (PRB == 3) {
+                                    if constexpr (F_BITS) asm volatile("" ::"v"(P.w[j]));
+                                    else asm volatile("" ::"v"(P.a[j]));
+                                    if constexpr (F_Z) asm volatile("" ::"v"(P.z[j]));
+                                }
+                            } else if constexpr (LOSS) {
+                                f32x4 tg;
+                                if constexpr (F_BITS) {
+                                    const uint32_t w = P.w[j] >> (n & 31);
+#pragma unroll
+                                    for (int e = 0; e < 4; ++e) tg[e] = (float)((w >> e) & 1u);
+                                } else {
+                                    tg = P.a[j];
+                                }
+#pragma unroll
+                                for (int e = 0; e < 4; ++e) {
+                                    o2[e] = v[e] + bias4[j][e];
+                                    o[e] = P.c1 * o2[e] - tg[e];
+                                    ss[p4] = fat_sq_add(ss[p4], o[e]);
+                                }
+                            } else {
+                                const f32x4 xt = P.a[j];
+#pragma unroll
+                                for (int e = 0; e < 4; ++e) {
+                                    float x0;
+                                    o[e] = fat_post_elem(v[e] + bias4[j][e], xt[e], F_Z ? P.z[j][e] : 0.f, P.c1, P.c2, P.p1, P.p2, P.sg, F_R, F_Z, x0);
+                                    o2[e] = x0;
+                                }
+                            }
+                            *reinterpret_cast<f32x4_e*>(g.C + m * g.ldc + n) = o;
+                            if constexpr (F_O2) *reinterpret_cast<f32x4_e*>(g.out2 + m * g.ldout2 + n) = o2;
+                        }
+                    }
+                    if constexpr (LOSS && PRB == 4) {
+#pragma unroll
+                        for (int p4 = 0; p4 < 4; ++p4) asm volatile("" ::"v"(ss[p4]));
+                    }
+                    if constexpr (LOSS && PRB >= 5) {
+#pragma unroll
+                        for (int p4 = 0; p4 < 4; ++p4) ss[p4] += fat_row_shl<1>(ss[p4]);
+#pragma unroll
+                        for (int p4 = 0; p4 < 4; ++p4) ss[p4] += fat_row_shl<2>(ss[p4]);
+#pragma unroll
+                        for (int p4 = 0; p4 < 4; ++p4) ss[p4] += fat_row_shl<4>(ss[p4]);
+#pragma unroll
+                        for (int p4 = 0; p4 < 4; ++p4) ss[p4] += fat_row_shl<8>(ss[p4]);
+                        if (r == 0) {
+#pragma unroll
+                            for (int p4 = 0; p4 < 4; ++p4) g.rowpart[(int64_t)(m0 + 16 * i + 4 * p4 + q) * g.ld_rowpart + tn] = ss[p4];
+                        }
+                    }
+                    __builtin_amdgcn_sched_barrier(0);
+                }
+                continue;
+            }
+        }
+
+        struct Pre {
+            f32x4 a[NJ], z[NJ];
+            uint32_t w[NJ];
+            float c1, c2, p1, p2, sg;
+        } pre[2];
+        auto fetch = [&](int i, int p4, Pre& P) {
+            const int mc = min(m0 + 16 * i + 4 * p4 + q, g.M - 1);
+            P.c1 = 1.f; P.c2 = 0.f; P.p1 = 0.f; P.p2 = 0.f; P.sg = 0.f;
+            if (EPI == GD_EPI_LOSS) {
+                if (g.r0) P.c1 = g.r0[mc];
+            } else {
+                P.c1 = g.r0[mc];
+                P.c2 = g.r1[mc];
+                if (has_r) { P.p1 = g.r2[mc]; P.p2 = g.r3[mc]; }
+                if (has_z) P.sg = g.r4[mc];
+            }
+#pragma unroll
+            for (int j = 0; j < NJ; ++j) {
+                const int n = col4[j];
+                const bool whole = (r + 16 * j < 4 * NB) && n + 3 < g.N;
+                P.w[j] = 0u;
+                P.a[j] = f32x4{0.f, 0.f, 0.f, 0.f};
+                P.z[j] = f32x4{0.f, 0.f, 0.f, 0.f};
+                if (bits) {
+                    P.w[j] = g.aux_bits[(int64_t)mc * g.ldbits + min((int64_t)(n >> 5), g.ldbits - 1)];
+                } else if (whole) {
+                    P.a[j] = *reinterpret_cast<const f32x4_e*>(g.aux + (int64_t)mc * g.ldaux + n);
+                    if (has_z) P.z[j] = *reinterpret_cast<const f32x4_e*>(g.aux2 + (int64_t)mc * g.ldaux2 + n);
+                }
+            }
+        };
+        fetch(0, 0, pre[0]);
+#pragma unroll
+        for (int i = 0; i < TMB; ++i) {
+#pragma unroll
+            for (int b = 0; b < NB; ++b)
+#pragma unroll
+                for (int t = 0; t < 4; ++t) lds[(4 * q + t) * LDS_ + 16 * b + r] = acc[i][b][t];
+            __builtin_amdgcn_sched_barrier(0);
+#pragma unroll
+            for (int p4 = 0; p4 < 4; ++p4) {
+                const int step = 4 * i + p4;
+                const Pre& P = pre[step & 1];
+                if (step + 1 < 4 * TMB) fetch((step + 1) >> 2, (step + 1) & 3, pre[(step + 1) & 1]);
+                const int m = m0 + 16 * i + 4 * p4 + q;
+                const int mc = min(m, g.M - 1);
+                const bool mok = m < g.M;
+                float ss = 0.f;
+                const float c1 = P.c1, c2 = P.c2, p1 = P.p1, p2 = P.p2, sg = P.sg;
+#pragma unroll
+                for (int j = 0; j < NJ; ++j) {
+                    const int c4 = r + 16 * j;
+                    const bool inb = c4 < 4 * NB;
+                    const int n = col4[j];
+                    const bool whole = inb && n + 3 < g.N;
+                    const bool full = whole && mok;
+                    const f32x4 v = *reinterpret_cast<const f32x4*>(lds + (4 * p4 + q) * LDS_ + 4 * min(c4, 4 * NB - 1));
+                    f32x4 o, o2 = f32x4{0.f, 0.f, 0.f, 0.f};
+                    if (EPI == GD_EPI_LOSS) {
+                        f32x4 tg;
+                        if (bits) {
+                            const uint32_t w = P.w[j] >> (n & 31);
+#pragma unroll
+                            for (int e = 0; e < 4; ++e) tg[e] = (float)((w >> e) & 1u);
+                        } else if (whole) {
+                            tg = P.a[j];
+                        } else {
+#pragma unroll
+                            for (int e = 0; e < 4; ++e) tg[e] = g.aux[(int64_t)mc * g.ldaux + min(n + e, g.N - 1)];
+                        }
+#pragma unroll
+                        for (int e = 0; e < 4; ++e) {
+                            o2[e] = v[e] + bias4[j][e];
+                            o[e] = c1 * o2[e] - tg[e];
+                            if (inb && mok && n + e < g.N) ss += o[e] * o[e];
+                        }
+                    } else {
+                        f32x4 xt = P.a[j], zz = P.z[j];
+                        if (!whole) {
+#pragma unroll
+                            for (int e = 0; e < 4; ++e) {
+                                xt[e] = g.aux[(int64_t)mc * g.ldaux + min(n + e, g.N - 1)];
+                                if (has_z) zz[e] = g.aux2[(int64_t)mc * g.ldaux2 + min(n + e, g.N - 1)];
+                            }
+                        }
+#pragma unroll
+                        for (int e = 0; e < 4; ++e) {
+                            const float vv = v[e] + bias4[j][e];
+                            if constexpr (GEN) {
+                                o2[e] = has_r ? (p1 * xt[e] - p2 * vv) : vv;
+                                o[e] = c1 * o2[e] + c2 * xt[e];
+                                if (has_z) o[e] += sg * zz[e];
+                            } else {
+                                float x0;
+                                o[e] = fat_post_elem(vv, xt[e], zz[e], c1, c2, p1, p2, sg, has_r, has_z, x0);
+                                o2[e] = x0;
+                            }
+                        }
+                    }
+                    if (full) {
+                        *reinterpret_cast<f32x4_e*>(g.C + (int64_t)m * g.ldc + n) = o;
+                        if (out2) *reinterpret_cast<f32x4_e*>(g.out2 + (int64_t)m * g.ldout2 + n) = o2;
+                    } else if (inb && mok) {
+                        for (int e = 0; e < 4 && n + e < g.N; ++e) {
+                            g.C[(int64_t)m * g.ldc + n + e] = o[e];
+                            if (out2) g.out2[(int64_t)m * g.ldout2 + n + e] = o2[e];
+                        }
+                    }
+                }
+                if (EPI == GD_EPI_LOSS) {
+                    ss += __shfl_xor(ss, 1);
+                    ss += __shfl_xor(ss, 2);
+                    ss += __shfl_xor(ss, 4);
+                    ss += __shfl_xor(ss, 8);
+                    if (r == 0 && mok) g.rowpart[(int64_t)m * g.ld_rowpart + tn] = ss;
+                }
+                __builtin_amdgcn_sched_barrier(0);
+            }
+        }
+    }
+}
+
+template <int NB, int EPI, int DMA, int FL>
+int dr_fat_start(const DrArgs& d, int n_cu, hipStream_t s) {
+    const size_t lds = (size_t)4 * 2 * NB * 256 * sizeof(float) + 4 * 64 * sizeof(float);
+    void (*kern)(const DrArgs) = dr_fat_kernel<NB, EPI, DMA, FL>;
+    static bool attr_set = false;
+    if (!attr_set && lds > 48 * 1024) {
+        hipError_t e = hipFuncSetAttribute(reinterpret_cast<const void*>(kern), hipFuncAttributeMaxDynamicSharedMemorySize, (int)lds);
+        if (e != hipSuccess) {
+            gdmcf_set_error("hipFuncSetAttribute(dr_fat_kernel, LDS=%zu): %s", lds, hipGetErrorString(e));
+            return GDMCF_E_HIP;
+        }
+        attr_set = true;
+    }
+    hipLaunchKernelGGL(kern, dim3(n_cu), dim3(256), lds, s, d);
+    return GDMCF_OK;
+}
+
+template <int EPI, int DMA, int FL>
+int dr_fat_start_nb(int nb, const DrArgs& d, int n_cu, hipStream_t s) {
+    switch (nb) {
+        case 8: return dr_fat_start<8, EPI, DMA, FL>(d, n_cu, s);
+        case 9: return dr_fat_start<9, EPI, DMA, FL>(d, n_cu, s);
+        case 10: return dr_fat_start<10, EPI, DMA, FL>(d, n_cu, s);
+        case 11: return dr_fat_start<11, EPI, DMA, FL>(d, n_cu, s);
+        default: return dr_fat_start<12, EPI, DMA, FL>(d, n_cu, s);
+    }
+}
+
+}
+
+int gd_dr_fat_loss_start(int nb, int fl, const void* d, int n_cu, hipStream_t s);
+int gd_dr_fat_post_start(int nb, int fl, const void* d, int n_cu, hipStream_t s);
+int gd_dr_fat_post2_start(int nb, int fl, const void* d, int n_cu, hipStream_t s);
diff --git a/gdmcf_amd/csrc/gemm_dr_fat_loss.hip b/gdmcf_amd/csrc/gemm_dr_fat_loss.hip
--- /dev/null
+++ b/gdmcf_amd/csrc/gemm_dr_fat_loss.hip
@@ -0,0 +1,6 @@
+#include "gemm_dr_fat_kernel.h"
+
+int gd_dr_fat_loss_start(int nb, int fl, const void* d, int n_cu, hipStream_t s) {
+    const DrArgs& a = *static_cast<const DrArgs*>(d);
+    return fl ? dr_fat_start_nb<GD_EPI_LOSS, 1, 1>(nb, a, n_cu, s) : dr_fat_start_nb<GD_EPI_LOSS, 1, 0>(nb, a, n_cu, s);
+}
diff --git a/gdmcf_amd/csrc/gemm_dr_fat_post.hip b/gdmcf_amd/csrc/gemm_dr_fat_post.hip
--- /dev/null
+++ b/gdmcf_amd/csrc/gemm_dr_fat_post.hip
@@ -0,0 +1,11 @@
+#include "gemm_dr_fat_kernel.h"
+
+int gd_dr_fat_post_start(int nb, int fl, const void* d, int n_cu, hipStream_t s) {
+    const DrArgs& a = *static_cast<const DrArgs*>(d);
+    switch (fl) {
+        case 0: return dr_fat_start_nb<GD_EPI_POST, 1, 0>(nb, a, n_cu, s);
+        case 1: return dr_fat_start_nb<GD_EPI_POST, 1, 1>(nb, a, n_cu, s);
+        case 2: return dr_fat_start_nb<GD_EPI_POST, 1, 2>(nb, a, n_cu, s);
+        default: return dr_fat_start_nb<GD_EPI_POST, 1, 3>(nb, a, n_cu, s);
+    }
+}
diff --git a/gdmcf_amd/csrc/gemm_dr_fat_post2.hip b/gdmcf_amd/csrc/gemm_dr_fat_post2.hip
--- /dev/null
+++ b/gdmcf_amd/csrc/gemm_dr_fat_post2.hip
@@ -0,0 +1,11 @@
+#include "gemm_dr_fat_kernel.h"
+
+int gd_dr_fat_post2_start(int nb, int fl, const void* d, int n_cu, hipStream_t s) {
+    const DrArgs& a = *static_cast<const DrArgs*>(d);
+    switch (fl) {
+        case 4: return dr_fat_start_nb<GD_EPI_POST, 1, 4>(nb, a, n_cu, s);
+        case 5: return dr_fat_start_nb<GD_EPI_POST, 1, 5>(nb, a, n_cu, s);
+        case 6: return dr_fat_start_nb<GD_EPI_POST, 1, 6>(nb, a, n_cu, s);
+        default: return dr_fat_start_nb<GD_EPI_POST, 1, 7>(nb, a, n_cu, s);
+    }
+}
```

Result: no change. 322,600 users/s, median of 6 (+0.4%).
